# mulns/AccFlow

Hardware: AMD Instinct MI355X
Metric: frame-pairs/s (estimator pair-evals/s), AccFlow(RAFT) 7-frame 480x1024 backward accumulation (higher is better)
Workload: dtype f32 (direct-kernel operands split into 2 fp16 terms - activations kept pre-split in HBM as fp16 hi+lo, 4 B per element; other kernels 3 bf16 terms; f32 accumulate); 1 GPU; AccFlow(RAFT) 7-frame 480x1024, 12 GRU iters, 1 sequence(s)/GPU/step (BASELINE.json configs[2]; configs[3] when n_gpus=8); parallelism=1 rank, no process group: no collective runs, weights=deterministic random init (no checkpoints offline)

## Files before the change

accflow_amd/build.py:

```python
import os
import subprocess
import sys
from concurrent.futures import ThreadPoolExecutor

HERE = os.path.dirname(os.path.abspath(__file__))
ROOT = os.path.dirname(HERE)
CSRC = os.path.join(HERE, "csrc")
LIBDIR = os.path.join(HERE, "lib")
LIB = os.path.join(LIBDIR, "libaccflow_hip.so")
SOURCES = ["conv2d_f32.hip", "conv2d_f32_v1.hip", "conv2d_f32_v2.hip", "conv2d_f32_v3.hip", "conv2d_bf16s.hip", "conv2d_bf16s_v12.hip", "conv2d_bf16s_v11.hip", "conv2d_bf16s_v21.hip",
           "conv2d_direct_v_bf16x6.hip", "conv2d_direct_v_bf16n.hip", "conv2d_direct_v_f16.hip", "conv2d_direct_v_s16.hip", "conv2d_direct_v_s16tg.hip", "conv2d_direct_v_s16k.hip", "conv2d_direct_v_s16k9.hip",
           "conv2d_direct_v_f16n.hip", "conv2d_direct_v_bf16x3.hip", "conv_s16m_v0.hip", "conv_s16m_v1.hip", "conv_s16m_v2.hip",
           "conv_s16m_v3.hip", "conv2d_s16m.hip", "conv_stem.hip", "conv2d_direct.hip", "conv2d.hip", "corr_volume.hip",
           "corr_lookup.hip", "corr_disp.hip", "corr_alt.hip", "corr_lookup_conv.hip", "sampling.hip", "misc.hip", "gma.hip", "backward.hip"]
ARCH = "gfx950"


def _hipcc():
    for c in (os.environ.get("HIPCC"), "/opt/rocm/bin/hipcc", "hipcc"):
        if c and (os.path.isabs(c) and os.path.exists(c) or not os.path.isabs(c)):
            return c
    raise RuntimeError("hipcc not found")


def _newer(target, deps):
    if not os.path.exists(target):
        return False
    t = os.path.getmtime(target)
    return all(os.path.getmtime(d) <= t for d in deps)


def _deps(src, seen=None):
    import re
    seen = set() if seen is None else seen
    if src in seen:
        return seen
    seen.add(src)
    for name in re.findall(r'^\s*#\s*include\s+"([^"]+)"', open(src).read(), flags=re.M):
        for d in (os.path.dirname(src), CSRC, os.path.join(ROOT, "include")):
            cand = os.path.join(d, name)
            if os.path.exists(cand):
                _deps(cand, seen)
                break
    return seen


def build(force=False, verbose=False, libdir=None, defines=(), unit_defines=()):
    LIBDIR = libdir or globals()["LIBDIR"]
    LIB = os.path.join(LIBDIR, "libaccflow_hip.so")
    os.makedirs(LIBDIR, exist_ok=True)
    objdir = os.path.join(LIBDIR, "obj")
    os.makedirs(objdir, exist_ok=True)
    cc = _hipcc()
    flags = ["-O3", "--offload-arch=" + ARCH, "-fPIC", "-std=c++17", "-I" + os.path.join(ROOT, "include"),
             "-I" + CSRC, "-Wno-unused-result",
             "-mllvm", "-pragma-unroll-threshold=1000000"] + ["-D" + d for d in defines]
    jobs = []
    objs = []
    for s in SOURCES:
        src = os.path.join(CSRC, s)
        obj = os.path.join(objdir, s.replace(".hip", ".o"))
        objs.append(obj)
        extra = ["-D" + d for pre, d in unit_defines if s.startswith(pre)]
        if force or extra or not _newer(obj, sorted(_deps(src))):
            jobs.append([cc] + flags + extra + ["-c", src, "-o", obj])

    def run(cmd):
        import time
        if verbose:
            print(" ".join(cmd), flush=True)
        t0 = time.time()
        r = subprocess.run(cmd, capture_output=True, text=True)
        if r.returncode != 0:
            raise RuntimeError("hipcc failed: %s\n%s\n%s" % (" ".join(cmd), r.stdout, r.stderr))
        if verbose:
            print("  [%.0f s] %s" % (time.time() - t0, os.path.basename(cmd[-1])), flush=True)

    if jobs:
        with ThreadPoolExecutor(max_workers=min(8, len(jobs))) as ex:
            list(ex.map(run, jobs))
    if jobs or force or not os.path.exists(LIB):
        run([cc, "--offload-arch=" + ARCH, "-shared", "-fPIC", "-no-hip-rt", "-o", LIB] + objs)
    return LIB


if __name__ == "__main__":
    defs = [a[2:] for a in sys.argv[1:] if a.startswith("-D")]
    ld = [a.split("=", 1)[1] for a in sys.argv[1:] if a.startswith("--libdir=")]
    ud = [tuple(a.split("=", 1)[1].split(":", 1)) for a in sys.argv[1:] if a.startswith("--unit-define=")]
    print(build(force="--force" in sys.argv, verbose=True, libdir=ld[0] if ld else None, defines=defs, unit_defines=ud))
```

accflow_amd/csrc/conv2d.hip:

```cpp
#include "conv_common.h"

namespace {

__global__ void conv_pack_patch_kernel(const float* __restrict__ w, const float* __restrict__ scale, int Cout, int Cin,
                                       int T, int CoutPad, unsigned short* __restrict__ wp, int f16,
                                       const float* __restrict__ wscale16, int octs = 2,
                                       const float* __restrict__ gptr = nullptr) {
  const int nstep = (Cin + 8 * octs - 1) / (8 * octs) * T;
  const long long per_term = (long long)nstep * octs * CoutPad * 8;
  const long long idx = (long long)blockIdx.x * blockDim.x + threadIdx.x;
  if (idx >= per_term) return;
  const int q = (int)(idx & 7);
  long long r = idx >> 3;
  const int ch = (int)(r % CoutPad); r /= CoutPad;
  const int o = (int)(r % octs); r /= octs;
  const int step = (int)r, cc = step / T, tap = step % T;
  const int c = cc * 8 * octs + o * 8 + q;
  float val = 0.0f;
  if (c < Cin && ch < Cout) {
    val = w[((long long)ch * Cin + c) * T + tap];
    if (scale) val *= scale[ch];
    if (gptr) val *= gptr[0];
  }
  float rr = val;
  if (f16) {
    rr = val * (ldexpf(1.0f, -ACCFLOW_F16_ASHIFT) / wscale16[ch]);
#pragma unroll
    for (int t = 0; t < 3; ++t) {
      const _Float16 hq = t < 2 ? (_Float16)rr : (_Float16)0.0f;
      wp[t * per_term + idx] = __builtin_bit_cast(unsigned short, hq);
      rr -= (float)hq;
    }
    return;
  }
#pragma unroll
  for (int t = 0; t < 3; ++t) {
    const __bf16 bq = (__bf16)rr;
    wp[t * per_term + idx] = __builtin_bit_cast(unsigned short, bq);
    rr -= (float)bq;
  }
}

__global__ void conv_pack_bf16s_kernel(const float* __restrict__ w, const float* __restrict__ scale, int Cout, int Cin,
                                       int KH, int KW, int Kpad, int CoutPad, unsigned short* __restrict__ ws,
                                       int kmajor, float cscale, const float* __restrict__ gptr,
                                       const float* __restrict__ wscale16 = nullptr) {
  const long long idx = (long long)blockIdx.x * blockDim.x + threadIdx.x;
  if (idx >= (long long)Kpad * CoutPad) return;
  w += (long long)blockIdx.y * Cout * Cin * KH * KW;
  ws += (long long)blockIdx.y * 3 * Kpad * CoutPad;
  if (wscale16) wscale16 += (long long)blockIdx.y * CoutPad;
  const int k = (int)(idx / CoutPad), o = (int)(idx % CoutPad);
  const int T = KH * KW, K = Cin * T;
  float val = 0.0f;
  if (k < K && o < Cout) {
    const int c = k / T, t = k % T;
    val = kmajor ? w[(long long)k * Cout + o] : w[((long long)o * Cin + c) * T + t];
    if (scale) val *= scale[o];
    val *= cscale;
    if (gptr) val *= gptr[0];
  }
  const long long per_term = (long long)Kpad * CoutPad;
  const long long dst = ((long long)(k / 8) * CoutPad + o) * 8 + (k % 8);
  float r = val;
  if (wscale16) {
    r = val * (ldexpf(1.0f, -ACCFLOW_F16_ASHIFT) / wscale16[o]);
#pragma unroll
    for (int t = 0; t < 3; ++t) {
      const _Float16 hq = t < 2 ? (_Float16)r : (_Float16)0.0f;
      ws[t * per_term + dst] = __builtin_bit_cast(unsigned short, hq);
      r -= (float)hq;
    }
    return;
  }
#pragma unroll
  for (int t = 0; t < 3; ++t) {
    const __bf16 b = (__bf16)r;
    ws[t * per_term + dst] = __builtin_bit_cast(unsigned short, b);
    r -= (float)b;
  }
}

__global__ __launch_bounds__(256) void conv_pack_kmajor_kernel(const float* __restrict__ w, int Cout, int K, int Kpad,
// ... 771 lines not shown
}

extern "C" long long accflow_s16_item_words(int C, int H, int W) {
  return (long long)((C + 7) / 8) * 2 * H * W * 4;
}

extern "C" int accflow_conv_kpad(int Cin, int KH, int KW) {
  const int K = Cin * KH * KW;
  return (K + 31) / 32 * 32;
}

extern "C" int accflow_conv_coutpad(int Cout) { return (Cout + 127) / 128 * 128; }

extern "C" int accflow_conv_pack_f32(const float* w, const float* scale, int Cout, int Cin, int KH, int KW,
                                     int C0, int tap_major, float* wpack, int* ktab, void* stream) {
  if (!w || !wpack || !ktab || Cout <= 0 || Cin <= 0 || KH <= 0 || KW <= 0) return 1;
  const int Kpad = accflow_conv_kpad(Cin, KH, KW), CoutPad = accflow_conv_coutpad(Cout);
  const long long n = (long long)Kpad * CoutPad;
  hipLaunchKernelGGL(conv_pack_kernel, dim3(cdiv(n, 256)), dim3(256), 0, as_stream(stream), w, scale, Cout,
                     Cin, KH, KW, C0, tap_major, Kpad, CoutPad, wpack, reinterpret_cast<int4*>(ktab));
  ACCFLOW_RETURN_LAUNCH_STATUS();
}

extern "C" int accflow_conv_pack_all_f32(const float* w, const float* scale, int Cout, int Cin, int KH, int KW, int C0, int tap_major,
                                         int transpose_flip, float* wpack, int* ktab, void* wsplit, void* wpatch, void* wpatch16,
                                         float* wscale16, void* wsplit16, void* stream) {
  if (!w || !wpack || !ktab || Cout <= 0 || Cin <= 0 || KH <= 0 || KW <= 0) return 1;
  if ((wpatch16 || wsplit16) && !wscale16) return 1;
  if (tap_major && (wsplit || wpatch || wpatch16 || wsplit16)) return 1;
  const int Kpad = accflow_conv_kpad(Cin, KH, KW), CoutPad = accflow_conv_coutpad(Cout);
  hipLaunchKernelGGL(conv_pack_all_kernel, dim3(CoutPad), dim3(256), 0, as_stream(stream), w, scale, Cout, Cin, KH, KW, C0, tap_major,
                     transpose_flip, Kpad, CoutPad, wpack, reinterpret_cast<int4*>(ktab), reinterpret_cast<unsigned short*>(wsplit),
                     reinterpret_cast<unsigned short*>(wpatch), reinterpret_cast<unsigned short*>(wpatch16), wscale16,
                     reinterpret_cast<unsigned short*>(wsplit16));
  ACCFLOW_RETURN_LAUNCH_STATUS();
}

thread_local int* accflow_tls_dry_slots = nullptr;
thread_local int* accflow_tls_dry_route = nullptr;

extern "C" int accflow_conv_in_norm_supported(const accflow_conv_desc* desc) {
  if (!desc) return 0;
  int slots = 0, route = 0;
  accflow_conv_desc probe = *desc;
  probe.in_norm = nullptr;
  probe.stats = nullptr;
  accflow_tls_dry_slots = &slots;
  accflow_tls_dry_route = &route;
  const int rc = accflow_conv2d_f32(&probe, nullptr);
  accflow_tls_dry_slots = nullptr;
  accflow_tls_dry_route = nullptr;
  return rc ? 0 : route;
}

extern "C" int accflow_conv_stat_slots(const accflow_conv_desc* desc) {
  if (!desc || desc->epi != ACCFLOW_EPI_STORE || desc->act != ACCFLOW_ACT_NONE) return 0;
  int slots = 0;
  accflow_tls_dry_slots = &slots;
  const int rc = accflow_conv2d_f32(desc, nullptr);
  accflow_tls_dry_slots = nullptr;
  return rc ? 0 : slots;
}

bool accflow_conv_stem_eligible(const accflow_conv_desc& d);
int accflow_launch_conv_stem(const accflow_conv_desc& d, hipStream_t st);

extern "C" int accflow_conv_gru16_supported(void) {
  static const bool ok = [] {
    const char* a = getenv("ACCFLOW_DIRECT_KT"); const char* b = getenv("ACCFLOW_DIRECT_W4"); const char* c = getenv("ACCFLOW_S16M");
    return !(a && atoi(a) == 0) && !(b && atoi(b) == 0) && !(c && atoi(c) != 0);
  }();
  return ok ? 1 : 0;
}

extern "C" int accflow_conv2d_f32(const accflow_conv_desc* desc, void* stream) {
  if (!desc) return 1;
  accflow_conv_desc dd = *desc;
  if (dd.mode == ACCFLOW_CONV_F16X3 && (dd.wpatch16 || dd.wsplit16) && !dd.wscale16) return 1;
  if (dd.mode != ACCFLOW_CONV_F16X3) { dd.wpatch16 = nullptr; dd.wsplit16 = nullptr; }
  if (!dd.wpatch16 && !dd.wsplit16) dd.wscale16 = nullptr;
  dd.acc_scale = 0.0f;
  if (dd.nsrc < 0 || dd.nsrc > ACCFLOW_CONV_MAX_SRC) return 1;
  const bool gru16 = !dd.nsrc && dd.e0_fmt;
  if (gru16 && !(dd.in_fmt == (dd.in1 ? 3 : 1) && dd.e0 && dd.pre && dd.out16 && dd.mode == ACCFLOW_CONV_F16X3 && !dd.cb && !dd.kws &&
                 dd.KH * dd.KW == 5 && dd.stride == 1 && accflow_conv_gru16_supported() && !dd.stats &&
                 ((dd.epi == ACCFLOW_EPI_GRU_ZR && dd.p32 == 3 && dd.out && dd.Cout == 256) ||
                  (dd.epi == ACCFLOW_EPI_GRU_Q && dd.p32 == 6 && dd.e1 && dd.Cout == 128))))
    return 1;
  if (!gru16 && dd.p32 && !(dd.p32 == 1 && !dd.nsrc && dd.in_fmt == (dd.in1 ? 3 : 1) && dd.mode == ACCFLOW_CONV_F16X3 && dd.out && !dd.out16 &&
                            dd.epi == ACCFLOW_EPI_STORE && (dd.act == ACCFLOW_ACT_NONE || dd.act == ACCFLOW_ACT_RELU) && !dd.cb &&
                            !dd.kws && !dd.stats && dd.stride == 1 && (dd.Cout % 128) == 0 && accflow_conv_gru16_supported()))
    return 1;
  const bool multi = dd.nsrc > 0;
  if (multi) {
    if (dd.mode != ACCFLOW_CONV_F16X3 || !dd.wpatch16 || dd.in_norm || dd.offset || dd.wsplit_bs) return 1;
    dd.in_fmt = 0; dd.in0 = nullptr; dd.in1 = nullptr; dd.H = dd.OH; dd.W = dd.OW;
    dd.CoutPad = accflow_conv_coutpad(dd.Cout);
  }
  const accflow_conv_desc& d = dd;
  if ((!multi && (!d.in0 || !d.wpack || !d.ktab)) || d.B <= 0 || d.Cout <= 0 || d.OH <= 0 || d.OW <= 0) return 1;
  if (d.epi == ACCFLOW_EPI_TAPGEMM) {
    if (multi || d.mode != ACCFLOW_CONV_F16X3 || !d.wpatch16 || !d.wscale16 || d.in_fmt != (d.in1 ? 3 : 1) || d.act != ACCFLOW_ACT_RELU ||
        (d.Cout & 127) || d.kws || d.stats || d.in_norm || d.cb || d.pre || d.offset || !d.tg_w16 || !d.tg_scale || !d.tg_out ||
        d.tg_rows < 1 || d.tg_rows > ACCFLOW_TAPGEMM_MAXROWS || d.tg_coutpad < 32 || (d.tg_coutpad & 31) ||
        d.tg_out_bs < (long long)d.tg_rows * d.OH * d.OW || (d.Cout > 128 && d.tg_out_ps <= 0) || !accflow_conv_direct_eligible(d) ||
        d.Kpad != accflow_conv_kpad(d.C0 + d.C1, d.KH, d.KW) || d.CoutPad != accflow_conv_coutpad(d.Cout))
      return 1;
    if ((((long long)(d.B - 1)) * d.in0_bs + accflow_s16_item_words(d.C0, d.H, d.W)) * 4 >= (1LL << 32)) return 1;
    if (d.in1 && (((long long)(d.B - 1)) * d.in1_bs + accflow_s16_item_words(d.C1, d.H, d.W)) * 4 >= (1LL << 32)) return 1;
    return accflow_launch_conv_direct(d, 2, as_stream(stream));
  }
  if (!d.out && (!d.out16 || d.epi == ACCFLOW_EPI_GRU_ZR)) return 1;
  if (d.epi == ACCFLOW_EPI_GRU_ZR && !d.out2 && !d.out16) return 1;
  if ((d.in_fmt || d.out16) && d.mode != ACCFLOW_CONV_F16X3) return 1;
  if (d.in_fmt & ~3) return 1;
  if (d.out16) {
    const int ea = d.epi * 8 + d.act;
    if (ea != ACCFLOW_EPI_STORE * 8 + ACCFLOW_ACT_NONE && ea != ACCFLOW_EPI_STORE * 8 + ACCFLOW_ACT_RELU &&
        ea != ACCFLOW_EPI_STORE * 8 + ACCFLOW_ACT_SIGMOID && ea != ACCFLOW_EPI_RES_RELU * 8 + ACCFLOW_ACT_RELU &&
        ea != ACCFLOW_EPI_RES_RELU * 8 + ACCFLOW_ACT_NONE &&
        ea != ACCFLOW_EPI_GRU_ZR * 8 + ACCFLOW_ACT_SIGMOID && ea != ACCFLOW_EPI_GRU_Q * 8 + ACCFLOW_ACT_TANH &&
        ea != ACCFLOW_EPI_ACCUM * 8 + ACCFLOW_ACT_NONE)
      return 1;
  }
  if (d.cb && ((d.cb & 31) || (d.epi != ACCFLOW_EPI_STORE && d.epi != ACCFLOW_EPI_ACCUM) || d.stats || d.Cout % d.cb)) return 1;
  if (!multi && (d.Kpad != accflow_conv_kpad(d.C0 + d.C1, d.KH, d.KW) || d.CoutPad != accflow_conv_coutpad(d.Cout))) return 1;
  if ((d.epi == ACCFLOW_EPI_RES_RELU || d.epi == ACCFLOW_EPI_ACCUM) && !d.e0) return 1;
  if (d.epi == ACCFLOW_EPI_GRU_ZR && (!d.e0 || (d.Cout & 1))) return 1;
  if (d.epi == ACCFLOW_EPI_GRU_ZR && d.out16 && ((d.Cout >> 1) & 7)) return 1;
  if (d.epi == ACCFLOW_EPI_GRU_Q && (!d.e0 || !d.e1)) return 1;
  if (d.pre && d.epi != ACCFLOW_EPI_GRU_ZR && d.epi != ACCFLOW_EPI_GRU_Q) return 1;
  if (d.offset && !d.dmask) return 1;
  if ((long long)d.B * d.OH * d.OW >= (1LL << 31)) return 1;
  if (!multi) {
    const long long w0 = (d.in_fmt & 1) ? accflow_s16_item_words(d.C0, d.H, d.W) : (long long)d.C0 * d.H * d.W;
    const long long w1 = (d.in_fmt & 2) ? accflow_s16_item_words(d.C1, d.H, d.W) : (long long)d.C1 * d.H * d.W;
    if ((((long long)(d.B - 1)) * d.in0_bs + w0) * 4 >= (1LL << 32)) return 1;
    if (d.in1 && (((long long)(d.B - 1)) * d.in1_bs + w1) * 4 >= (1LL << 32)) return 1;
  }
  if (d.out16 && (((long long)(d.B - 1)) * d.out16_bs + accflow_s16_item_words(d.Cout, d.OH, d.OW)) * 4 >= (1LL << 32)) return 1;
  if (d.stats && (d.epi != ACCFLOW_EPI_STORE || d.act != ACCFLOW_ACT_NONE || d.stat_slots <= 0)) return 1;
  hipStream_t st = as_stream(stream);
  const long long Ptot = (long long)d.B * d.OH * d.OW;
  if (d.in_norm && !accflow_tls_dry_slots && !accflow_conv_in_norm_supported(&d)) return 1;
  if (d.stats && !accflow_tls_dry_slots) {
    int want = 0;
    accflow_tls_dry_slots = &want;
    accflow_conv_desc probe = d;
    probe.stats = nullptr;
    const int prc = accflow_conv2d_f32(&probe, nullptr);
    accflow_tls_dry_slots = nullptr;
    if (prc || want != d.stat_slots) return 1;
  }
  if (multi) return accflow_launch_conv_s16m(d, -1, st);
  static const bool stem_on = [] { const char* e = getenv("ACCFLOW_CONV_STEM"); return !e || atoi(e) != 0; }();
  if (stem_on && accflow_conv_stem_eligible(d)) return accflow_launch_conv_stem(d, st);
  static const bool s16m_on = [] { const char* e = getenv("ACCFLOW_S16M"); return e && atoi(e) != 0; }();
  if (d.in_fmt && s16m_on) {
    if (!accflow_conv_direct_eligible(d) || !d.wpatch16 || d.in_norm) return 1;
    if (d.in_fmt != (d.in1 ? 3 : 1)) return 1;
    accflow_conv_desc e = d;
    accflow_s16m_from_legacy(e);
    return accflow_launch_conv_s16m(e, -1, st);
  }
  if (d.in_fmt || d.out16 || d.cb) {
    if (!accflow_conv_direct_eligible(d) || !d.wpatch16 || d.stats || d.in_norm) return 1;
    if (d.in_fmt && d.in_fmt != (d.in1 ? 3 : 1)) return 1;
    return accflow_launch_conv_direct(d, d.Cout > 64 ? 2 : 1, st);
  }
  if (d.Cout <= 4 && !d.offset && (d.epi == ACCFLOW_EPI_STORE || d.epi == ACCFLOW_EPI_ACCUM || d.epi == ACCFLOW_EPI_RES_RELU)) {
    const bool same = d.stride == 1 && d.OH == d.H && d.OW == d.W && d.KH * d.KW >= 2 && d.C0 + d.C1 >= 16 &&
                      (8 + d.KH - 1) * (16 + d.KW - 1) <= 192 && d.KH * d.KW <= 25 && (!d.in1 || d.C0 % 16 == 0);
    ACCFLOW_DRY_RUN(0);
    if (same) {
      dim3 pgrid((unsigned)((long long)d.B * cdiv(d.OW, 16) * cdiv(d.OH, 8)));
      if (d.Cout <= 2) hipLaunchKernelGGL((conv2d_small_cout_patch_kernel<2>), pgrid, dim3(256), 0, st, d);
      else hipLaunchKernelGGL((conv2d_small_cout_patch_kernel<4>), pgrid, dim3(256), 0, st, d);
      ACCFLOW_RETURN_LAUNCH_STATUS();
    }
    dim3 grid(cdiv(Ptot, 64));
    if (d.Cout <= 2) hipLaunchKernelGGL((conv2d_small_cout_kernel<2>), grid, dim3(256), 0, st, d);
    else hipLaunchKernelGGL((conv2d_small_cout_kernel<4>), grid, dim3(256), 0, st, d);
    ACCFLOW_RETURN_LAUNCH_STATUS();
  }
  if (accflow_conv_direct_eligible(d)) {
    const long long nb = (long long)d.B * cdiv(d.OW, DIR_TW) * cdiv(d.OH, DIR_TH);
    const long long minb = (d.kws && (d.KH * d.KW >= 2 || d.C0 + d.C1 >= 512)) ? 0 : patch_min_blocks();
    if (d.Cout > 64 && nb * cdiv(d.Cout, 128) >= minb) return accflow_launch_conv_direct(d, 2, st);
    if (nb * cdiv(d.Cout, 64) >= minb) return accflow_launch_conv_direct(d, 1, st);
  }
  if (d.mode == ACCFLOW_CONV_F16X3 && !(d.wsplit16 && !d.offset && d.Cout > 32)) {
    accflow_conv_desc e = d;
    e.mode = ACCFLOW_CONV_BF16X6;
    e.wpatch = nullptr;
    e.wpatch16 = nullptr; e.wsplit16 = nullptr; e.wscale16 = nullptr;
    return accflow_conv2d_f32(&e, stream);
  }
  if (d.mode == ACCFLOW_CONV_F16X3 && d.wsplit_bs) {
    ACCFLOW_DRY_RUN(0);
    if ((d.OH * d.OW) % 64) return 1;
    return d.Cout > 64 ? accflow_launch_conv_bf16s(d, 2, 1, st) : accflow_launch_conv_bf16s(d, 1, 1, st);
  }
  if (d.mode == ACCFLOW_CONV_F16X3) {
    accflow_conv_desc e = d;
    e.wpatch16 = nullptr;
    auto nb = [&](int bc, int bp) { return (long long)cdiv(Ptot, bp) * cdiv(e.Cout, bc); };
    if (e.Cout <= 64) return nb(64, 128) >= 384 ? accflow_launch_conv_bf16s(e, 1, 2, st) : accflow_launch_conv_bf16s(e, 1, 1, st);
    if (nb(128, 128) >= 384) return accflow_launch_conv_bf16s(e, 2, 2, st);
    if (nb(128, 64) >= 384) return accflow_launch_conv_bf16s(e, 2, 1, st);
    return accflow_launch_conv_bf16s(e, 1, 1, st);
  }
  if (d.wsplit_bs) {
    ACCFLOW_DRY_RUN(0);
    if (d.mode == ACCFLOW_CONV_F32 || !d.wsplit || d.offset || ((d.OH * d.OW) % 64) || d.Cout <= 32) return 1;
// ... 27 lines not shown
```

accflow_amd/csrc/conv2d_direct.hip:

```cpp
#include "conv2d_direct_kernel.h"

namespace {

__global__ __launch_bounds__(256) void conv_ksplit_reduce_kernel(const accflow_conv_desc d, int Z) {
  const int OHW = d.OH * d.OW;
  const long long n = (long long)d.B * d.Cout * OHW;
  const long long i = (long long)blockIdx.x * 256 + threadIdx.x;
  if (i >= n) return;
  const int px = (int)(i % OHW);
  const int ch = (int)((i / OHW) % d.Cout);
  const int b = (int)(i / ((long long)OHW * d.Cout));
  float v = d.kws[i];
  for (int z = 1; z < Z; ++z) v += d.kws[(long long)z * n + i];
  v = fmaf(v, d.wscale16 ? d.wscale16[(d.wsplit_bs ? (long long)b * d.CoutPad : 0) + ch] : 1.0f, d.bias ? d.bias[ch] : 0.0f);
  if (d.pre && (d.epi == ACCFLOW_EPI_GRU_ZR || d.epi == ACCFLOW_EPI_GRU_Q)) v += d.pre[b * d.pre_bs + (long long)ch * OHW + px];
  v = apply_act(v, d.act);
  const long long o = (long long)ch * OHW + px;
  const int half = d.Cout >> 1;
  if (d.cb) {
    const int blk = ch / d.cb;
    const long long oc = (long long)(ch - blk * d.cb) * OHW + px;
    const float r = d.epi == ACCFLOW_EPI_ACCUM ? d.e0[b * d.e0_bs + blk * d.e0_cbs + oc] + v : v;
    d.out[b * d.out_bs + blk * d.out_cbs + oc] = r;
    return;
// ... 143 lines not shown
      } break;
      case ACCFLOW_EPI_ACCUM: t = d.e0[b * d.e0_bs + o] + t; break;
      default: break;
    }
    if (d.out) d.out[b * d.out_bs + o] = t;
    res[j] = t;
  }
  constexpr float ASC = (float)(1 << ACCFLOW_F16_ASHIFT);
  unsigned hi[2], lo[2];
  bool bad = false;
#pragma unroll
  for (int k = 0; k < 2; ++k) {
    const float a = res[2 * k] * ASC, c = res[2 * k + 1] * ASC;
    bad |= !(fabsf(a) < 65520.0f) | !(fabsf(c) < 65520.0f);
    const f32x2 v2 = {a, c};
    const f16x2 hq = __builtin_convertvector(v2, f16x2);
    const f32x2 back = __builtin_convertvector(hq, f32x2);
    const f32x2 rest = {a - back[0], c - back[1]};
    const f16x2 lq = __builtin_convertvector(rest, f16x2);
    hi[k] = __builtin_bit_cast(unsigned, hq);
    lo[k] = __builtin_bit_cast(unsigned, lq);
  }
  unsigned* base = reinterpret_cast<unsigned*>(d.out16) + b * d.out16_bs;
  int oct = q >> 1;
  const int w0 = (q & 1) * 2;
  if (d.cb) {
    base += (long long)((q * 4) / d.cb) * d.out16_cbs;
    oct = ((q * 4) % d.cb) >> 3;
  }
  unsigned* ph = base + (((long long)(oct * 2 + 0)) * OHW + px) * 4 + w0;
  unsigned* pl = base + (((long long)(oct * 2 + 1)) * OHW + px) * 4 + w0;
  typedef unsigned u2_ __attribute__((ext_vector_type(2)));
  *reinterpret_cast<u2_*>(ph) = u2_{hi[0], hi[1]};
  *reinterpret_cast<u2_*>(pl) = u2_{lo[0], lo[1]};
  if (bad && d.guard) atomicOr(d.guard, 1);
}

}

int conv_ksplit_reduce_launch(const accflow_conv_desc& d, int Z, hipStream_t st) {
  if (d.out16 && !(d.Cout & 7) && !(d.cb & 7) && d.epi != ACCFLOW_EPI_GRU_ZR) {
    const long long nthr = (long long)d.B * (d.Cout / 4) * d.OH * d.OW;
    hipLaunchKernelGGL(conv_ksplit_reduce_s16q_kernel, dim3(cdiv(nthr, 256)), dim3(256), 0, st, d, Z);
  } else if (d.out16) {
    const long long nthr = (long long)d.B * ((d.Cout + 7) / 8) * d.OH * d.OW;
    hipLaunchKernelGGL(conv_ksplit_reduce_s16_kernel, dim3(cdiv(nthr, 256)), dim3(256), 0, st, d, Z);
  } else {
    const long long nout = (long long)d.B * d.Cout * d.OH * d.OW;
    hipLaunchKernelGGL(conv_ksplit_reduce_kernel, dim3(cdiv(nout, 256)), dim3(256), 0, st, d, Z);
  }
  ACCFLOW_RETURN_LAUNCH_STATUS();
}

namespace {

template <int TC>
int launch_conv_direct(const accflow_conv_desc& d, hipStream_t st) {
  const int tiles = cdiv(d.OW, DIR_TW) * cdiv(d.OH, DIR_TH);
  const long long nb = (long long)d.B * tiles * cdiv(d.Cout, 2 * TC * 32);
  static const bool w4 = [] { const char* e = getenv("ACCFLOW_DIRECT_W4"); return !e || atoi(e) != 0; }();
  const bool norm_ok = !d.in1 && d.C0 <= DIR_NORM_MAXC && (TC == 1 || w4);
  if (accflow_tls_dry_route) *accflow_tls_dry_route = norm_ok ? 1 : 0;
  ACCFLOW_DRY_RUN(tiles * ((TC == 2 && w4) ? 1 : 2));
  if (d.in_norm && !norm_ok) return 1;
  int Z = 1;
  const long long nout = (long long)d.B * d.Cout * d.OH * d.OW;
  const int nchunk = (d.C0 + d.C1 + 15) / 16;
  if (d.kws && nchunk >= 256 && nb < 700 && !d.stats) {
    static const int zenv = [] { const char* e = getenv("ACCFLOW_DIRECT_KSPLIT"); return e ? atoi(e) : 0; }();
    double best = 0.0;
    for (int z = 1; z <= 8; ++z) {
      const double fill = (double)(nb * z) / (double)(cdiv(nb * z, 768) * 768);
      if (fill > best + 0.03) { best = fill; Z = z; }
    }
    if (zenv > 0) Z = zenv;
  } else if (d.kws && nb < 320 && !d.stats) {
    Z = (int)((512 + nb - 1) / nb);
    if (Z > 4) Z = 4;
    if (Z > nchunk / 2) Z = nchunk / 2;
  }
  if (Z > 1 && (long long)Z * nout > d.kws_elems) Z = (int)(d.kws_elems / nout);
  if (Z < 1) Z = 1;
  if (d.out16 && d.epi == ACCFLOW_EPI_GRU_ZR && ((d.Cout >> 1) & 7)) Z = 1;
  dim3 grid((unsigned)((long long)d.B * tiles), cdiv(d.Cout, 2 * TC * 32), Z);
  constexpr bool CAN_W4 = TC == 2;
  const bool f16 = d.mode == ACCFLOW_CONV_F16X3 && d.wpatch16;
  int rc;
  if (d.epi == ACCFLOW_EPI_TAPGEMM) {
    if (TC != 2 || !f16 || !d.in_fmt || Z != 1 || !(CAN_W4 && w4)) return 1;
    static const bool kt9_tg = [] { const char* e = getenv("ACCFLOW_DIRECT_KT9"); return !e || atoi(e) != 0; }();
    rc = (kt9_tg && d.KH == 3 && d.KW == 3 && (d.C0 + d.C1) % 16 == 0) ? accflow_direct_launch_s16k9(d, 2, true, grid, st)
                                                                        : accflow_direct_launch_s16tg(d, grid, st);
  } else if (d.in_fmt) {
    if (!f16 || d.in_norm || d.in_fmt != (d.in1 ? 3 : 1)) return 1;
    static const bool kt_on = [] { const char* e = getenv("ACCFLOW_DIRECT_KT"); return !e || atoi(e) != 0; }();
    static const bool kt9_on = [] { const char* e = getenv("ACCFLOW_DIRECT_KT9"); return !e || atoi(e) != 0; }();
    if (kt_on && TC == 2 && CAN_W4 && w4 && d.KH * d.KW == 5) rc = accflow_direct_launch_s16k(d, 5, grid, st);
    else if (kt9_on && (TC == 1 || (CAN_W4 && w4)) && d.KH == 3 && d.KW == 3) rc = accflow_direct_launch_s16k9(d, TC, false, grid, st);
    else rc = accflow_direct_launch_s16(d, TC, grid, st);
  } else if (d.in_norm) {
    rc = f16 ? accflow_direct_launch_f16_norm(d, TC, grid, st)
             : accflow_direct_launch_bf16_norm(d, TC, d.mode == ACCFLOW_CONV_BF16X3 ? 2 : 3, grid, st);
  } else {
    rc = f16 ? accflow_direct_launch_f16(d, TC, CAN_W4 && w4, grid, st)
             : accflow_direct_launch_bf16(d, TC, d.mode == ACCFLOW_CONV_BF16X3 ? 2 : 3, CAN_W4 && w4, grid, st);
  }
  if (rc) return rc;
  if (Z > 1) return conv_ksplit_reduce_launch(d, Z, st);
  ACCFLOW_RETURN_LAUNCH_STATUS();
}

}

template <int NT, bool F16>
__global__ __launch_bounds__(256, 2) void corr_disp_gemm_kernel(const accflow_conv_desc d) {
  constexpr int TC = 2, TP = 2;
  __shared__ __attribute__((aligned(16))) unsigned char smem[DISP2_LDS_BYTES];
#ifdef ACCFLOW_KPROF
  const unsigned long long tL0 = __builtin_amdgcn_s_memrealtime();
#endif
  const int tid = threadIdx.x, lane = tid & 63;
  const int wave = __builtin_amdgcn_readfirstlane(tid >> 6);
  const int wc = wave >> 1, wp = wave & 1;
  const int l31 = lane & 31, kh = lane >> 5;
  const int P = d.OH * d.OW;
  const int npb = (P + 127) >> 7, percol = (npb + 7) >> 3;
  const int xcd = blockIdx.x & 7, seq = blockIdx.x >> 3;
  const int pb = xcd + 8 * (seq % percol), qt = seq / percol;
  if (pb >= npb) return;
  const int ncx = (d.OW + 63) >> 6;
  const int yo = qt / ncx, xc = qt - yo * ncx;
  const int cblk0 = pb * 128;
  const int nstep = d.Kpad / 16;
  const long long step_bytes = 2LL * d.CoutPad * 16, term_bytes = (long long)(d.Kpad / 8) * d.CoutPad * 16;
  const __amdgpu_buffer_rsrc_t ra = __builtin_amdgcn_make_buffer_rsrc(
      const_cast<void*>(F16 ? d.wpatch16 : d.wpatch), 0, (int)(unsigned)(3 * term_bytes), 0x00020000);
  const __amdgpu_buffer_rsrc_t rb = __builtin_amdgcn_make_buffer_rsrc(
      const_cast<float*>(d.in0), 0, (int)(unsigned)(3 * term_bytes), 0x00020000);
  const unsigned avoff = (unsigned)((kh * d.CoutPad + cblk0 + wc * 64 + l31) * 16);
  unsigned bvoff[2];
#pragma unroll
  for (int i = 0; i < 2; ++i) {
    const int y2 = 2 * yo + wp, x2 = xc * 64 + i * 32 + l31;
    bvoff[i] = (y2 < d.OH && x2 < d.OW) ? (unsigned)((kh * d.CoutPad + y2 * d.OW + x2) * 16) : 0xFFFFFFFFu;
  }
#define CG_LOAD(STEP, A, Bf)                                                                                     \
  _Pragma("unroll") for (int t = 0; t < NT; ++t) _Pragma("unroll") for (int i = 0; i < 2; ++i) {                 \
    const int so = (int)(unsigned)(t * term_bytes + (STEP) * step_bytes);                                        \
    A[t][i] = __builtin_bit_cast(bf16x8, __builtin_amdgcn_raw_buffer_load_b128(ra, (int)(avoff + i * 512), so, 0)); \
    Bf[t][i] = __builtin_bit_cast(bf16x8, __builtin_amdgcn_raw_buffer_load_b128(rb, (int)bvoff[i], so, 0));      \
  }
  f32x16 acc[TC][TP];
#pragma unroll
  for (int tc = 0; tc < TC; ++tc)
#pragma unroll
    for (int tp = 0; tp < TP; ++tp)
#pragma unroll
      for (int r = 0; r < 16; ++r) acc[tc][tp][r] = 0.0f;
  constexpr int PD = NT == 2 ? 2 : 1;
  bf16x8 aA[NT][TC], bA[NT][TP], aB[NT][TC], bB[NT][TP], aC[NT][TC], bC[NT][TP];
  CG_LOAD(0, aA, bA);
  if (PD == 2 && nstep > 1) { CG_LOAD(1, aB, bB); }
#define CG_STEP(STEP, AC, BC, AN, BN)                                                                            \
  do {                                                                                                           \
    if ((STEP) + PD < nstep) { CG_LOAD((STEP) + PD, AN, BN); }                                                   \
    constexpr int NPAIR = NT == 3 ? 6 : 3;                                                                       \
// ... 282 lines not shown
    constexpr int PA[3] = {1, 0, 0}, PB[3] = {0, 1, 0};
#pragma unroll
    for (int pr = 0; pr < 3; ++pr)
#pragma unroll
      for (int tc = 0; tc < TC; ++tc)
#pragma unroll
        for (int tp = 0; tp < TP; ++tp) {
          if (ACCFLOW_CORR_ABL & 2) acc[tc][tp][pr] += __builtin_bit_cast(float, __builtin_bit_cast(u32x4, A[PA[pr]][tc])[0] ^ __builtin_bit_cast(u32x4, Bf[PB[pr]][tp])[1]);
          else acc[tc][tp] = dir_mfma<true>(A[PA[pr]][tc], Bf[PB[pr]][tp], acc[tc][tp]);
        }
  }
  __syncthreads();
  if ((ACCFLOW_CORR_ABL & 8) && acc[0][0][0] != 12345.678f) return;
#ifdef ACCFLOW_KPROF
  __builtin_amdgcn_sched_barrier(0);
  const unsigned long long tL1 = __builtin_amdgcn_s_memrealtime();
#endif
  corr_disp_store2(d, acc, reinterpret_cast<float*>(smem), reinterpret_cast<int*>(smem) + 64 * DISP_PITCH,
                   reinterpret_cast<float*>(smem + DISP_LDS_BYTES), d.out2, cblk0, yo, xc, wc, wp, lane, wave, tid);
#ifdef ACCFLOW_KPROF
  __builtin_amdgcn_sched_barrier(0);
  const unsigned long long tL2 = __builtin_amdgcn_s_memrealtime();
  asm volatile("s_waitcnt vmcnt(0)" ::: "memory");
  if (tid == 0) {
    const int slot = (blockIdx.x & 4095) * 16;
    g_kprof[slot + 8] = tL1 - tL0;
    g_kprof[slot + 9] = tL2 - tL1;
    g_kprof[slot + 11] = __builtin_amdgcn_s_memrealtime() - tL0;
    g_kprof[slot + 10] = 1;
  }
#endif
}

int accflow_launch_corr_disp_direct(const accflow_conv_desc& d, hipStream_t st) {
  const int P = d.OH * d.OW, npb = cdiv(P, 128);
  if (!d.out2) return 1;
  const int nqt = cdiv(d.OH, 2) * cdiv(d.OW, 64);
  dim3 grid(8 * ((npb + 7) / 8) * nqt);
  static const bool ringk = [] { const char* e = getenv("ACCFLOW_CORR_GEMM"); return !(e && e[0] == 'r'); }();
  if (d.mode == ACCFLOW_CONV_F16X3 && d.wpatch16 && ringk) {
    hipLaunchKernelGGL(corr_disp_ring_kernel, grid, dim3(256), 0, st, d);
  } else if (d.mode == ACCFLOW_CONV_F16X3 && d.wpatch16) hipLaunchKernelGGL((corr_disp_gemm_kernel<2, true>), grid, dim3(256), 0, st, d);
  else if (d.mode == ACCFLOW_CONV_BF16X3) hipLaunchKernelGGL((corr_disp_gemm_kernel<2, false>), grid, dim3(256), 0, st, d);
  else hipLaunchKernelGGL((corr_disp_gemm_kernel<3, false>), grid, dim3(256), 0, st, d);
  ACCFLOW_RETURN_LAUNCH_STATUS();
}

int accflow_launch_conv_direct(const accflow_conv_desc& d, int tc, hipStream_t st) {
  const bool pointwise = d.epi == ACCFLOW_EPI_STORE || d.epi == ACCFLOW_EPI_RES_RELU || d.epi == ACCFLOW_EPI_ACCUM;
  if (tc == 2 && d.Cout > 128 && d.Cout % 128 > 0 && d.Cout % 128 <= 64 && pointwise && !d.stats && !accflow_tls_dry_slots && !(d.kws && (long long)d.B * cdiv(d.OW, DIR_TW) * cdiv(d.OH, DIR_TH) * cdiv(d.Cout, 128) < 320)) {
    const int ch0 = d.Cout / 128 * 128;
    const long long OHW = (long long)d.OH * d.OW;
    accflow_conv_desc a = d, b = d;
    a.Cout = ch0;
    b.Cout = d.Cout - ch0;
    b.out = d.out ? d.out + ch0 * OHW : nullptr;
    if (d.bias) b.bias = d.bias + ch0;
    if (d.wscale16) b.wscale16 = d.wscale16 + ch0;
    if (d.e0) b.e0 = d.e0 + ch0 * OHW;
    if (d.out16) b.out16 = reinterpret_cast<char*>(d.out16) + (long long)(ch0 / 8) * 2 * OHW * 16;
    if (d.wpatch) b.wpatch = reinterpret_cast<const char*>(d.wpatch) + (long long)ch0 * 16;
    if (d.wpatch16) b.wpatch16 = reinterpret_cast<const char*>(d.wpatch16) + (long long)ch0 * 16;
    const int rc = launch_conv_direct<2>(a, st);
    if (rc) return rc;
    return launch_conv_direct<1>(b, st);
  }
  return tc == 2 ? launch_conv_direct<2>(d, st) : launch_conv_direct<1>(d, st);
}

bool accflow_conv_direct_eligible(const accflow_conv_desc& d) {
  if (!d.wpatch || d.wsplit_bs || d.mode == ACCFLOW_CONV_F32 || d.offset || d.stride != 1 || d.Cout <= 4) return false;
  if (d.OH != d.H || d.OW != d.W) return false;
  if ((DIR_TH + d.KH - 1) * (DIR_TW + d.KW - 1) > DIR_NPMAX) return false;
  if (d.C0 + d.C1 < 16) return false;
  if (d.in1 && (d.C0 % (d.KH * d.KW == 1 ? 32 : 16))) return false;
  return true;
}

#ifdef ACCFLOW_KPROF
#define ACCFLOW_DIRECT_UNITY
#include "conv2d_direct_v_s16.hip"
#include "conv2d_direct_v_s16tg.hip"
#include "conv2d_direct_v_s16k.hip"
#include "conv2d_direct_v_s16k9.hip"
#include "conv2d_direct_v_f16.hip"
#include "conv2d_direct_v_f16n.hip"
#include "conv2d_direct_v_bf16x6.hip"
#include "conv2d_direct_v_bf16x3.hip"
#include "conv2d_direct_v_bf16n.hip"
extern "C" int accflow_debug_occupancy(int* out) {
  int n = 0;
  hipOccupancyMaxActiveBlocksPerMultiprocessor(&out[n++], conv2d_direct_bf16s_kernel<2, 3>, 256, 0);
  hipOccupancyMaxActiveBlocksPerMultiprocessor(&out[n++], conv2d_direct_bf16s_kernel<2, 2, true>, 256, 0);
  hipOccupancyMaxActiveBlocksPerMultiprocessor(&out[n++], conv2d_direct_bf16s_kernel<1, 3>, 256, 0);
  hipDeviceProp_t pr; hipGetDeviceProperties(&pr, 0);
  out[n++] = (int)(pr.maxSharedMemoryPerMultiProcessor / 1024); out[n++] = (int)(pr.sharedMemPerBlock / 1024);
  out[n++] = pr.regsPerMultiprocessor; out[n++] = pr.regsPerBlock;
  return n;
}
extern "C" int accflow_debug_kprof(unsigned long long* out, int reset) {
  hipDeviceSynchronize();
  hipMemcpyFromSymbol(out, HIP_SYMBOL(g_kprof), 4096 * 16 * 8);
  if (reset) { void* p; hipGetSymbolAddress(&p, HIP_SYMBOL(g_kprof)); hipMemset(p, 0, 4096 * 16 * 8); }
  return (int)hipGetLastError();
}
#endif
```

accflow_amd/csrc/conv2d_direct_kernel.h:

```cpp
#pragma once
#include "conv_common.h"
#include <utility>

namespace {


#ifndef ACCFLOW_DIRECT_LEAN
#define ACCFLOW_DIRECT_LEAN 1
#endif
#ifndef ACCFLOW_DIRECT_LEAN_MAXSTEPS
#define ACCFLOW_DIRECT_LEAN_MAXSTEPS 0
#endif
#ifndef ACCFLOW_F16_PAIRMASK
#define ACCFLOW_F16_PAIRMASK 7
#endif
#ifndef ACCFLOW_DIRECT_KT_BUPFRONT
#define ACCFLOW_DIRECT_KT_BUPFRONT 0
#endif
#ifndef ACCFLOW_DIRECT_KT_WAVES
#define ACCFLOW_DIRECT_KT_WAVES 3
#endif
#ifndef ACCFLOW_DIRECT_SETPRIO
#define ACCFLOW_DIRECT_SETPRIO 0
#endif
// ... 33 lines not shown
template <bool F16, class PixMap>
__device__ __forceinline__ void conv_epilogue_tapgemm(const accflow_conv_desc& d, f32x16 (&acc)[1][4], int cblk0, int wave,
                                                      int lane, int tid, int OHW, PixMap pixmap, float* red) {
  typedef float f32x4_ __attribute__((ext_vector_type(4)));
  typedef float f32x2_ __attribute__((ext_vector_type(2)));
  typedef _Float16 f16x2_ __attribute__((ext_vector_type(2)));
  const int l31 = lane & 31, kh = lane >> 5, lh4 = kh * 4;
  const int rowbase = cblk0 + wave * 32;
  const int R = d.tg_rows;
  const __amdgpu_buffer_rsrc_t r_b = __builtin_amdgcn_make_buffer_rsrc(const_cast<float*>(d.bias ? d.bias : d.wscale16), 0,
                                                                      d.bias ? d.Cout * 4 : 0, 0x00020000);
  const __amdgpu_buffer_rsrc_t r_s = __builtin_amdgcn_make_buffer_rsrc(const_cast<float*>(d.wscale16), 0, d.CoutPad * 4, 0x00020000);
  f32x4_ bv[4], sv[4];
#pragma unroll
  for (int m = 0; m < 4; ++m) {
    const int off = (rowbase + 8 * m + lh4) * 4;
    bv[m] = __builtin_bit_cast(f32x4_, __builtin_amdgcn_raw_buffer_load_b128(r_b, off, 0, 0));
    sv[m] = __builtin_bit_cast(f32x4_, __builtin_amdgcn_raw_buffer_load_b128(r_s, off, 0, 0));
  }
  const long long step_bytes2 = 2LL * d.tg_coutpad * 16, term_bytes2 = (long long)(d.Cout >> 4) * step_bytes2;
  const __amdgpu_buffer_rsrc_t r_w2 = __builtin_amdgcn_make_buffer_rsrc(const_cast<void*>(d.tg_w16), 0,
                                                                       (int)(unsigned)(2 * term_bytes2), 0x00020000);
  const unsigned av2 = (unsigned)((kh * d.tg_coutpad + l31) * 16);
  bf16x8 a2[2][2];
#pragma unroll
  for (int s = 0; s < 2; ++s)
#pragma unroll
    for (int t = 0; t < 2; ++t)
      a2[s][t] = __builtin_bit_cast(bf16x8, __builtin_amdgcn_raw_buffer_load_b128(
                                               r_w2, (int)av2, (int)(unsigned)(t * term_bytes2 + ((rowbase >> 4) + s) * step_bytes2), 0));
  constexpr float ASC16 = (float)(1 << ACCFLOW_F16_ASHIFT);
  bool bad16 = false;
#pragma unroll
  for (int tp = 0; tp < 4; ++tp) {
    f32x16 z2;
#pragma unroll
    for (int r = 0; r < 16; ++r) z2[r] = 0.0f;
#pragma unroll
    for (int s = 0; s < 2; ++s) {
      unsigned hi[4], lo[4];
#pragma unroll
      for (int e2 = 0; e2 < 4; ++e2) {
        const int m = 2 * s + (e2 >> 1), q = (2 * e2) & 3;
        float va = fmaf(acc[0][tp][4 * m + q], sv[m][q], bv[m][q]) + 0.0f;
        float vb = fmaf(acc[0][tp][4 * m + q + 1], sv[m][q + 1], bv[m][q + 1]) + 0.0f;
        va = fmaxf(va, 0.0f) * ASC16;
        vb = fmaxf(vb, 0.0f) * ASC16;
        bad16 |= !(va < 65520.0f) | !(vb < 65520.0f);
        const f32x2_ v2 = {va, vb};
        const f16x2_ hq = __builtin_convertvector(v2, f16x2_);
        const f32x2_ back = __builtin_convertvector(hq, f32x2_);
        const f32x2_ rest = {va - back[0], vb - back[1]};
        const f16x2_ lq = __builtin_convertvector(rest, f16x2_);
        hi[e2] = __builtin_bit_cast(unsigned, hq);
        lo[e2] = __builtin_bit_cast(unsigned, lq);
      }
      const u32x4 hv = {hi[0], hi[1], hi[2], hi[3]}, lv = {lo[0], lo[1], lo[2], lo[3]};
      const bf16x8 bh = __builtin_bit_cast(bf16x8, hv), bl = __builtin_bit_cast(bf16x8, lv);
      z2 = dir_mfma<F16>(a2[s][1], bh, z2);
      z2 = dir_mfma<F16>(a2[s][0], bl, z2);
      z2 = dir_mfma<F16>(a2[s][0], bh, z2);
    }
#pragma unroll
    for (int r = 0; r < 16; ++r) {
      const int row = 8 * (r >> 2) + lh4 + (r & 3);
      if (row < R) red[(wave * R + row) * (DIR_TH * DIR_TW) + tp * 32 + l31] = z2[r];
    }
  }
  if (bad16 && d.guard) atomicOr(d.guard, 1);
  __syncthreads();
  const long long obase = (long long)(cblk0 >> 7) * d.tg_out_ps;
  constexpr int NPX = DIR_TH * DIR_TW;
  for (int o = tid; o < R * NPX; o += 256) {
    const int row = o / NPX, px = o - row * NPX;
    const float v = ((red[o] + red[R * NPX + o]) + red[2 * R * NPX + o]) + red[3 * R * NPX + o];
    int b;
    const int rem = pixmap(px, b);
    if (rem >= 0) d.tg_out[obase + (long long)b * d.tg_out_bs + (long long)row * OHW + rem] = v * d.tg_scale[row];
  }
}

constexpr int DIR_NORM_MAXC = 256;
template <int TC, int NT, bool F16 = false, bool W4 = false, bool NORM = false, bool S16 = false, int PM = 7, bool TG = false, int KT = 0,
          int KWC = 0>
__global__ __launch_bounds__(256, (KT == 5 ? ACCFLOW_DIRECT_KT_WAVES : 2)) void conv2d_direct_bf16s_kernel(const accflow_conv_desc d) {
  static_assert(!F16 || NT == 2, "the fp16 split has two terms");
  static_assert(KT == 0 || ((S16 || (F16 && NORM)) && (KT & 1)), "the tap-specialised loop: S16 sources or the fp16 normalise-on-load gather, an odd tap count");
  static_assert(!TG || (W4 && S16 && PM == 7), "ACCFLOW_EPI_TAPGEMM: the 4 x 1 wave layout over S16 sources");
  static_assert(!W4 || TC == 2, "the 4 x 1 wave layout is the 128-channel kernel's");
  static_assert(!S16 || (F16 && !NORM), "S16 sources hold the fp16 split");
#ifdef ACCFLOW_KPROF
  const unsigned long long tL0 = __builtin_amdgcn_s_memrealtime();
  unsigned long long kp[8] = {0, 0, 0, 0, 0, 0, 0, 0};
#endif
  constexpr int WC = W4 ? 4 : 2, WP = W4 ? 1 : 2, TP = W4 ? 4 : 2, OCT = 2;
  constexpr int TCW = W4 ? 1 : TC;
  constexpr int BC = WC * TCW * 32;
  static_assert(BC == 2 * TC * 32 && DIR_TH * DIR_TW == WP * TP * 32, "4 x 32 pixel tile = 128 accumulator columns");
  constexpr int PSTAGE = NT * OCT * DIR_NPMAX;
  constexpr int TGWORDS = TG ? 4 * ACCFLOW_TAPGEMM_MAXROWS * DIR_TH * DIR_TW / 4 : 0;
  __shared__ u32x4 Pst[2 * PSTAGE > TGWORDS ? 2 * PSTAGE : TGWORDS];
  __shared__ float Nrm[NORM ? 2 * DIR_NORM_MAXC : 2];

  const int tid = threadIdx.x, lane = tid & 63;
  const int wave = __builtin_amdgcn_readfirstlane(tid >> 6);
  const int wc = wave / WP, wp = wave % WP;
  const int l31 = lane & 31, kh = lane >> 5;
  int bx = blockIdx.x, by = blockIdx.y;
#if ACCFLOW_CONV_XCD_ORDER
  if (gridDim.y > 1 && (d.C0 + d.C1) * d.KH * d.KW >= ACCFLOW_CONV_XCD_MIN_K) {
    const int X = gridDim.x, Y = gridDim.y, L = bx + X * by, full = X & ~7;
    if (L < full * Y) {
      const int G = L / (8 * Y), r = L - G * 8 * Y;
      by = r >> 3;
      bx = G * 8 + (r & 7);
    } else {
      const int r = L - full * Y, rem = X - full;
      by = r / rem;
      bx = full + r - by * rem;
    }
  }
#endif
  const int cblk0 = by * BC;
  const int OHW = d.OH * d.OW;
  const int tilesX = (d.OW + DIR_TW - 1) / DIR_TW, tilesY = (d.OH + DIR_TH - 1) / DIR_TH;
  const int tb = bx / (tilesX * tilesY), trem = bx - tb * tilesX * tilesY;
  const int oy0 = (trem / tilesX) * DIR_TH, ox0 = (trem % tilesX) * DIR_TW;
#ifdef ACCFLOW_DIRECT_STAGGER
  if (KT == 5 && (blockIdx.x & 1)) {
    for (int i = 0; i < ACCFLOW_DIRECT_STAGGER; ++i) __builtin_amdgcn_s_sleep(127);
  }
#endif
  const int T = d.KH * d.KW;
  const int PW = DIR_TW + d.KW - 1, NP = (DIR_TH + d.KH - 1) * PW;
  const int Cin = d.C0 + d.C1;
  const bool wide = T == 1;
  const int CCH = wide ? 32 : 16;
  const int NOCT = wide ? 4 : 2;
  const int NPS = wide ? DIR_NPMAX / 2 : DIR_NPMAX;
  const int TPC = wide ? 2 : T;
  const int nstep = (Cin + 15) / 16 * T, nchunk = (Cin + CCH - 1) / CCH;
  const int HW = d.H * d.W;
  const int c_begin = (int)((long long)nchunk * blockIdx.z / gridDim.z);
  const int c_end = (int)((long long)nchunk * (blockIdx.z + 1) / gridDim.z);
  const int step_end = min(c_end * TPC, nstep);

  unsigned voff0[2], voff1[2];
  int p_oct[2], p_pix[2];
#pragma unroll
  for (int i = 0; i < 2; ++i) {
    const int it = tid + 256 * i;
    const bool live = it < NOCT * NP;
    p_oct[i] = live ? it / NP : 0;
    p_pix[i] = live ? it - p_oct[i] * NP : 0;
    const int py = p_pix[i] / PW, px = p_pix[i] - py * PW;
    const int iy = oy0 - d.padH + py, ix = ox0 - d.padW + px;
    const bool ok = live && (unsigned)iy < (unsigned)d.H && (unsigned)ix < (unsigned)d.W;
    voff0[i] = ok ? (unsigned)(((long long)tb * d.in0_bs + iy * d.W + ix) * 4) : 0xFFFFFFFFu;
    voff1[i] = ok ? (unsigned)(((long long)tb * d.in1_bs + iy * d.W + ix) * 4) : 0xFFFFFFFFu;
    if (!live) p_pix[i] = -1;
  }
  const __amdgpu_buffer_rsrc_t rsrc0 = __builtin_amdgcn_make_buffer_rsrc(
      const_cast<float*>(d.in0), 0, (int)(unsigned)((((long long)(d.B - 1)) * d.in0_bs + (long long)d.C0 * HW) * 4),
      0x00020000);
  const __amdgpu_buffer_rsrc_t rsrc1 = __builtin_amdgcn_make_buffer_rsrc(
      const_cast<float*>(d.in1 ? d.in1 : d.in0), 0,
      (int)(unsigned)(d.in1 ? (((long long)(d.B - 1)) * d.in1_bs + (long long)d.C1 * HW) * 4 : 0), 0x00020000);
  unsigned pixo[4] = {0xFFFFFFFFu, 0xFFFFFFFFu, 0xFFFFFFFFu, 0xFFFFFFFFu};
  const int O0 = (d.C0 + 7) >> 3, O1 = (d.C1 + 7) >> 3;
  const __amdgpu_buffer_rsrc_t rs16_0 = __builtin_amdgcn_make_buffer_rsrc(
      const_cast<float*>(d.in0), 0, (int)(unsigned)((((long long)(d.B - 1)) * d.in0_bs + (long long)O0 * 2 * HW * 4) * 4),
      0x00020000);
  const __amdgpu_buffer_rsrc_t rs16_1 = __builtin_amdgcn_make_buffer_rsrc(
      const_cast<float*>(d.in1 ? d.in1 : d.in0), 0,
      (int)(unsigned)(d.in1 ? (((long long)(d.B - 1)) * d.in1_bs + (long long)O1 * 2 * HW * 4) * 4 : 0), 0x00020000);
  if constexpr (S16) {
#pragma unroll
    for (int q = 0; q < 4; ++q) {
      const int pp = q * 64 + lane;
      const int py = pp / PW, px = pp - py * PW;
      const int iy = oy0 - d.padH + py, ix = ox0 - d.padW + px;
      const bool ok = pp < NP && (unsigned)iy < (unsigned)d.H && (unsigned)ix < (unsigned)d.W;
      pixo[q] = ok ? (unsigned)(iy * d.W + ix) * 16u : 0xFFFFFFFFu;
    }
  }
  auto issue_dma = [&](int stage, int cc) {
    const int c0 = cc * CCH;
    const bool second = c0 >= d.C0;
    const int cs = second ? c0 - d.C0 : c0, osrc = second ? O1 : O0;
    const long long bs = second ? d.in1_bs : d.in0_bs;
    const unsigned item = (unsigned)((long long)tb * bs * 4);
#pragma unroll
    for (int i = 0; i < 4; ++i) {
      const int row = wide ? 2 * wave + (i >> 1) : wave;
      const int q = wide ? (i & 1) : i;
      if (!wide && q * 64 >= NP) continue;
      const int t = wide ? row >> 2 : row >> 1, o = wide ? row & 3 : row & 1;
      const int oct = (cs >> 3) + o;
      const unsigned soff = (unsigned)__builtin_amdgcn_readfirstlane((int)(item + (unsigned)((oct * 2 + t) * HW) * 16u));
      const unsigned voff = oct < osrc ? (q == 0 ? pixo[0] : q == 1 ? pixo[1] : q == 2 ? pixo[2] : pixo[3]) : 0xFFFFFFFFu;
      const int slot = __builtin_amdgcn_readfirstlane(stage * PSTAGE + t * (OCT * DIR_NPMAX) + o * NPS + q * 64);
      if (second)
        __builtin_amdgcn_raw_ptr_buffer_load_lds(rs16_1, (__attribute__((address_space(3))) void*)&Pst[slot], 16, (int)voff,
                                                 (int)soff, 0, 0);
      else
        __builtin_amdgcn_raw_ptr_buffer_load_lds(rs16_0, (__attribute__((address_space(3))) void*)&Pst[slot], 16, (int)voff,
                                                 (int)soff, 0, 0);
    }
  };
  float xa[8], xb[8];
  unsigned vq0[2], vq1[2];
#pragma unroll
  for (int i = 0; i < 2; ++i) {
    const unsigned po = (unsigned)p_oct[i] * 8u * (unsigned)HW * 4u;
    vq0[i] = voff0[i] != 0xFFFFFFFFu ? voff0[i] + po : 0xFFFFFFFFu;
    vq1[i] = voff1[i] != 0xFFFFFFFFu ? voff1[i] + po : 0xFFFFFFFFu;
  }
  auto gather_patch = [&](int cc) {
    const int c0 = cc * CCH;
    const bool second = c0 >= d.C0;
    const __amdgpu_buffer_rsrc_t rs = second ? rsrc1 : rsrc0;
    const int cs = second ? c0 - d.C0 : c0, cmax = second ? d.C1 : d.C0;
    if (cs + CCH <= cmax) {
      const unsigned va = second ? vq1[0] : vq0[0], vb = second ? vq1[1] : vq0[1];
      const unsigned so = (unsigned)__builtin_amdgcn_readfirstlane(cs) * (unsigned)HW * 4u;
#pragma unroll
      for (int q = 0; q < 8; ++q) {
        const int sq = (int)(so + (unsigned)q * (unsigned)HW * 4u);
        xa[q] = __builtin_bit_cast(float, __builtin_amdgcn_raw_buffer_load_b32(rs, (int)va, sq, 0));
        xb[q] = __builtin_bit_cast(float, __builtin_amdgcn_raw_buffer_load_b32(rs, (int)vb, sq, 0));
      }
      return;
    }
#pragma unroll
    for (int q = 0; q < 8; ++q) {
      const int ca = cs + p_oct[0] * 8 + q, cb = cs + p_oct[1] * 8 + q;
      const unsigned va = second ? voff1[0] : voff0[0], vb = second ? voff1[1] : voff0[1];
      const unsigned oa = (ca < cmax && va != 0xFFFFFFFFu) ? va + (unsigned)ca * (unsigned)HW * 4u : 0xFFFFFFFFu;
      const unsigned ob = (cb < cmax && vb != 0xFFFFFFFFu) ? vb + (unsigned)cb * (unsigned)HW * 4u : 0xFFFFFFFFu;
      xa[q] = __builtin_bit_cast(float, __builtin_amdgcn_raw_buffer_load_b32(rs, (int)oa, 0, 0));
      xb[q] = __builtin_bit_cast(float, __builtin_amdgcn_raw_buffer_load_b32(rs, (int)ob, 0, 0));
    }
  };
  bool bad = false;
  constexpr float ASC = (float)(1 << ACCFLOW_F16_ASHIFT);
  if constexpr (NORM) {
    for (int i = tid; i < 2 * d.C0; i += 256) Nrm[i] = d.in_norm[(long long)tb * 2 * d.C0 + i];
    __syncthreads();
  }
  auto store_patch = [&](int stage, int cc) {
    if constexpr (NORM) {
      const int ca = cc * CCH + p_oct[0] * 8, cb = cc * CCH + p_oct[1] * 8;
      const bool ina = voff0[0] != 0xFFFFFFFFu, inb = voff0[1] != 0xFFFFFFFFu;
#pragma unroll
      for (int q = 0; q < 8; ++q) {
        const bool oka = ina && ca + q < d.C0, okb = inb && cb + q < d.C0;
        const float ma = Nrm[2 * min(ca + q, d.C0 - 1)], ra = Nrm[2 * min(ca + q, d.C0 - 1) + 1];
        const float mb = Nrm[2 * min(cb + q, d.C0 - 1)], rb = Nrm[2 * min(cb + q, d.C0 - 1) + 1];
        xa[q] = oka ? fmaxf((xa[q] - ma) * ra, 0.0f) : 0.0f;
        xb[q] = okb ? fmaxf((xb[q] - mb) * rb, 0.0f) : 0.0f;
      }
    }
    u32x4 terms[NT];
    if constexpr (F16) split8_f16<0>(xa, terms, bad, ASC);
    else split8_bf16<NT, 0>(xa, terms);
    if (p_pix[0] >= 0) {
#pragma unroll
      for (int t = 0; t < NT; ++t) Pst[stage * PSTAGE + t * (OCT * DIR_NPMAX) + p_oct[0] * NPS + p_pix[0]] = terms[t];
    }
    if constexpr (F16) split8_f16<0>(xb, terms, bad, ASC);
    else split8_bf16<NT, 0>(xb, terms);
    if (p_pix[1] >= 0) {
#pragma unroll
      for (int t = 0; t < NT; ++t) Pst[stage * PSTAGE + t * (OCT * DIR_NPMAX) + p_oct[1] * NPS + p_pix[1]] = terms[t];
    }
  };

  const long long step_bytes = 2LL * d.CoutPad * 16, term_bytes = (long long)nstep * step_bytes;
  const __amdgpu_buffer_rsrc_t rsrcw = __builtin_amdgcn_make_buffer_rsrc(const_cast<void*>(F16 ? d.wpatch16 : d.wpatch), 0,
                                                                        (int)(unsigned)(3 * term_bytes), 0x00020000);
  const unsigned avoff = (unsigned)((kh * d.CoutPad + cblk0 + wc * TCW * 32 + l31) * 16);
#define DIR_LOAD_A(STEP, A)                                                                                      \
  _Pragma("unroll") for (int t = 0; t < NT; ++t) _Pragma("unroll") for (int tc = 0; tc < TCW; ++tc)              \
      A[t][tc] = __builtin_bit_cast(bf16x8, __builtin_amdgcn_raw_buffer_load_b128(                              \
          rsrcw, (int)(avoff + tc * 512), (int)(unsigned)(t * term_bytes + (STEP) * step_bytes), 0))

  int pbase[TP];
#pragma unroll
  for (int tp = 0; tp < TP; ++tp) pbase[tp] = (wp * TP + tp) * PW + l31;

  f32x16 acc[TCW][TP];
#pragma unroll
  for (int tc = 0; tc < TCW; ++tc)
#pragma unroll
    for (int tp = 0; tp < TP; ++tp)
#pragma unroll
      for (int r = 0; r < 16; ++r) acc[tc][tp][r] = 0.0f;

  bf16x8 aA[NT][TCW], aB[NT][TCW];
  DIR_LOAD_A(c_begin * TPC, aA);
  if constexpr (S16) {
    issue_dma(c_begin & 1, c_begin);
    asm volatile("s_waitcnt vmcnt(0)" ::: "memory");
  } else {
    gather_patch(c_begin);
    store_patch(c_begin & 1, c_begin);
  }
  __syncthreads();

  int cc = c_begin, tap = 0, ty = 0, tx = 0;
#define DIR_STEP(STEP, ACUR, ANXT)                                                                               \
  do {                                                                                                           \
    KPROF_T(tA);                                                                                                 \
    const int pstage = cc & 1;                                                                                   \
    const bool next_chunk = cc + 1 < c_end;                                                                      \
    if ((STEP) + 1 < step_end) { DIR_LOAD_A((STEP) + 1, ANXT); }                                                 \
    if (tap == 0 && next_chunk) {                                                                                \
      if constexpr (S16) issue_dma(pstage ^ 1, cc + 1); else gather_patch(cc + 1);                               \
    }                                                                                                            \
    KPROF_T(tA1);                                                                                                \
    const int toff = wide ? tap * 2 * NPS : ty * PW + tx;                                                        \
    bf16x8 b[NT][TP];                                                                                            \
    _Pragma("unroll") for (int t = 0; t < NT; ++t) _Pragma("unroll") for (int tp = 0; tp < TP; ++tp)             \
        b[t][tp] = __builtin_bit_cast(bf16x8, Pst[pstage * PSTAGE + t * (OCT * DIR_NPMAX) + kh * NPS + pbase[tp] + toff]); \
    KPROF_T(tB);                                                                                                 \
    KPROF_WAIT();                                                                                                \
    KPROF_T(tB2);                                                                                                \
    {                                                                                                            \
      if (ACCFLOW_DIRECT_SETPRIO) __builtin_amdgcn_s_setprio(ACCFLOW_DIRECT_SETPRIO);                            \
      constexpr int NPAIR = NT == 3 ? 6 : 3;                                                                     \
      constexpr int PA[6] = {2, 0, 1, 1, 0, 0}, PB[6] = {0, 2, 1, 0, 1, 0};                                      \
      _Pragma("unroll") for (int pr = 6 - NPAIR; pr < 6; ++pr) _Pragma("unroll") for (int tc = 0; tc < TCW; ++tc) \
          _Pragma("unroll") for (int tp = 0; tp < TP; ++tp) if (!F16 || (((ACCFLOW_F16_PAIRMASK & PM) >> (pr - 3)) & 1))  \
              acc[tc][tp] = dir_mfma<F16>(ACUR[PA[pr]][tc], b[PB[pr]][tp], acc[tc][tp]);                         \
      if (ACCFLOW_DIRECT_SETPRIO) __builtin_amdgcn_s_setprio(0);                                                 \
    }                                                                                                            \
    KPROF_T(tC);                                                                                                 \
    if (++tx == d.KW) { tx = 0; ++ty; }                                                                          \
    if (++tap == TPC || (STEP) + 1 == step_end) {                                                                \
      if constexpr (S16) { asm volatile("s_waitcnt vmcnt(0)" ::: "memory"); }                                    \
      else { if (next_chunk) store_patch(pstage ^ 1, cc + 1); }                                                  \
      KPROF_T(tD);                                                                                               \
      __syncthreads();                                                                                           \
      KPROF_T(tE);                                                                                               \
      KPROF_ACC(3, tD - tC); KPROF_ACC(4, tE - tD);                                                              \
      tap = 0; ty = 0; tx = 0; ++cc;                                                                             \
    }                                                                                                            \
    KPROF_ACC(0, tA1 - tA); KPROF_ACC(7, tB - tA1); KPROF_ACC(1, tB2 - tB); KPROF_ACC(2, tC - tB2); KPROF_ACC(5, 1); \
  } while (0)

#ifdef ACCFLOW_KPROF
  const unsigned long long tK0 = __builtin_readcyclecounter();
  const unsigned long long tR0 = __builtin_amdgcn_s_memrealtime();
  if (tid == 0) KP_SLOT(14) = tR0 - tL0;
#endif
  if constexpr (KT > 0) {
    static_assert(KWC > 0 && KT % KWC == 0, "the tap-specialised loop knows the kernel's width");
    constexpr int PWC_ = DIR_TW + KWC - 1;
    s16m_i32x4 wdesc;
    {
      const unsigned long long wp_ = (unsigned long long)(F16 ? d.wpatch16 : d.wpatch);
      wdesc[0] = (int)(unsigned)wp_;
      wdesc[1] = (int)(unsigned)((wp_ >> 32) & 0xFFFFu);
      wdesc[2] = (int)(unsigned)(3 * term_bytes);
      wdesc[3] = 0x00020000;
    }
    constexpr int NPC = (DIR_TH + KT / KWC - 1) * PWC_;
    constexpr int NDMA = !S16 ? 16 : (NPC + 63) / 64 < 4 ? (NPC + 63) / 64 : 4;
    auto load_a_asm = [&](int step, bf16x8 (&A)[NT][TCW]) __attribute__((always_inline)) {
#pragma unroll
      for (int t = 0; t < NT; ++t)
#pragma unroll
        for (int tc = 0; tc < TCW; ++tc)
        {
          u32x4 frag;
          s16m_load_a(frag, avoff + tc * 512, wdesc,
                      __builtin_amdgcn_readfirstlane((int)(unsigned)(t * term_bytes + (long long)step * step_bytes)));
          A[t][tc] = __builtin_bit_cast(bf16x8, frag);
        }
    };
    constexpr int PWC = DIR_TW + KWC - 1;
    const u32x4* const pb0 = &Pst[kh * DIR_NPMAX + wp * TP * PWC + l31];
    auto chunk = [&](int cq, bf16x8 (&A0)[NT][TCW], bf16x8 (&A1)[NT][TCW]) __attribute__((always_inline)) {
      const int pstage = cq & 1;
      const bool next_chunk = cq + 1 < c_end;
      const int sbase = cq * KT;
      const u32x4* const pb = pb0 + pstage * PSTAGE;
      dir_static_for<KT>([&](auto tap_) {
        constexpr int TAP = decltype(tap_)::value;
        bf16x8 (&ACUR)[NT][TCW] = (TAP & 1) ? A1 : A0;
        bf16x8 (&ANXT)[NT][TCW] = (TAP & 1) ? A0 : A1;
        const int snext = sbase + TAP + 1;
        if constexpr (TAP + 1 < KT) { load_a_asm(snext, ANXT); }
        else { if (next_chunk) { load_a_asm(snext, ANXT); } }
        if constexpr (TAP == 0) {
          if (next_chunk) {
            if constexpr (S16) issue_dma(pstage ^ 1, cq + 1);
            else gather_patch(cq + 1);
          }
        }
        bf16x8 b[NT][TP];
#pragma unroll
        for (int tt = 0; tt < NT; ++tt)
#pragma unroll
          for (int tp = 0; tp < TP; ++tp)
            b[tt][tp] = __builtin_bit_cast(bf16x8, pb[tt * (OCT * DIR_NPMAX) + tp * PWC + (TAP / KWC) * PWC + TAP % KWC]);
        constexpr int PA[3] = {1, 0, 0}, PB[3] = {0, 1, 0};
#pragma unroll
        for (int pr = 0; pr < 3; ++pr)
#pragma unroll
          for (int tc = 0; tc < TCW; ++tc)
#pragma unroll
            for (int tp = 0; tp < TP; ++tp) acc[tc][tp] = dir_mfma<F16>(ACUR[PA[pr]][tc], b[PB[pr]][tp], acc[tc][tp]);
#if ACCFLOW_DIRECT_KT_BUPFRONT
        __builtin_amdgcn_sched_group_barrier(0x100, NT * TP, 0);
        __builtin_amdgcn_sched_group_barrier(0x008, 3 * TCW * TP, 0);
#endif
        __builtin_amdgcn_sched_barrier(0);
        if constexpr (TAP == 0 && KT > 1) { if (next_chunk) s16m_wait_vm<NDMA>(); else s16m_wait_vm<0>(); }
        else if constexpr (TAP + 1 < KT) { s16m_wait_vm<0>(); }
      });
      s16m_wait_vm<0>();
      if constexpr (!S16) { if (next_chunk) store_patch(pstage ^ 1, cq + 1); }
      __syncthreads();
    };
    for (int cq = c_begin; cq < c_end; cq += 2) {
      chunk(cq, aA, aB);
      if (cq + 1 < c_end) chunk(cq + 1, aB, aA);
    }
  } else {
  for (int step = c_begin * TPC; step < step_end; step += 2) {
    DIR_STEP(step, aA, aB);
    if (step + 1 < step_end) DIR_STEP(step + 1, aB, aA);
  }
  }
#undef DIR_STEP
#undef DIR_LOAD_A
#ifdef ACCFLOW_KPROF
  {
    const unsigned long long tK1 = __builtin_readcyclecounter();
    if (tid == 0) {
      for (int i = 0; i < 6; ++i) KP_SLOT(i) = kp[i];
      KP_SLOT(6) = tK1 - tK0;
      KP_SLOT(7) = kp[7];
      KP_SLOT(8) = __builtin_amdgcn_s_memrealtime() - tR0;
      KP_SLOT(10) = 1;
    }
  }
#endif
  if constexpr (F16) {
    if (bad && d.guard) atomicOr(d.guard, 1);
  }
  auto pixmap = [&](int j, int& b) {
    const int oy = oy0 + j / DIR_TW, ox = ox0 + j % DIR_TW;
    b = tb;
    return (oy < d.OH && ox < d.OW) ? oy * d.OW + ox : -1;
  };
  if constexpr (TG) {
    conv_epilogue_tapgemm<F16>(d, acc, cblk0, wave, lane, tid, OHW, pixmap, reinterpret_cast<float*>(Pst));
    return;
  }
  if (gridDim.z > 1) {
    accflow_conv_desc e = d;
    e.out = d.kws + (long long)blockIdx.z * d.B * d.Cout * OHW;
    e.out_bs = (long long)d.Cout * OHW;
    e.bias = nullptr;
    e.wscale16 = nullptr;
    e.out16 = nullptr;
    e.cb = 0;
    conv_epilogue_impl<ACCFLOW_EPI_STORE, ACCFLOW_ACT_NONE, WC, WP, TCW, TP>(e, acc, cblk0, wc, wp, lane, OHW, pixmap);
    return;
  }
  if constexpr (S16) {
    if ((ACCFLOW_DIRECT_LEAN || d.p32 || nstep <= ACCFLOW_DIRECT_LEAN_MAXSTEPS) && d.epi == ACCFLOW_EPI_STORE && !d.cb && !d.stats && cblk0 + (wc + 1) * TCW * 32 <= d.Cout &&
        (d.act == ACCFLOW_ACT_NONE || d.act == ACCFLOW_ACT_RELU)) {
      if (d.act == ACCFLOW_ACT_RELU) conv_epilogue_lean<ACCFLOW_ACT_RELU, WC, WP, TCW, TP>(d, acc, cblk0, wc, wp, lane, OHW, pixmap);
      else conv_epilogue_lean<ACCFLOW_ACT_NONE, WC, WP, TCW, TP>(d, acc, cblk0, wc, wp, lane, OHW, pixmap);
      return;
    }
  }
#ifdef ACCFLOW_DIRECT_ABL_NOEPI
  if ((d.epi == ACCFLOW_EPI_GRU_ZR || d.epi == ACCFLOW_EPI_GRU_Q) && acc[0][0][0] != 12345.678f) return;
#endif
  if constexpr (S16 && W4 && KT == 5) {
    if (d.e0_fmt) {
      if (d.epi == ACCFLOW_EPI_GRU_ZR) conv_epilogue_gru16<true, TP>(d, acc, cblk0, wc, lane, OHW, pixmap);
      else conv_epilogue_gru16<false, TP>(d, acc, cblk0, wc, lane, OHW, pixmap);
      return;
    }
  }
  conv_epilogue_px<WC, WP, TCW, TP, decltype(pixmap), F16>(d, acc, cblk0, wc, wp, lane, OHW, pixmap, tb, trem * WP + wp);
#ifdef ACCFLOW_KPROF
  __builtin_amdgcn_sched_barrier(0);
  const unsigned long long tS = __builtin_amdgcn_s_memrealtime();
  asm volatile("s_waitcnt vmcnt(0)" ::: "memory");
  if (tid == 0) {
    KP_SLOT(15) = tS - tL0;
    KP_SLOT(11) = __builtin_amdgcn_s_memrealtime() - tL0;
  }
#endif
}


}

int accflow_direct_launch_s16(const accflow_conv_desc& d, int tc, dim3 grid, hipStream_t st);
int accflow_direct_launch_s16tg(const accflow_conv_desc& d, dim3 grid, hipStream_t st);
int accflow_direct_launch_s16k9(const accflow_conv_desc& d, int tc, bool tapgemm, dim3 grid, hipStream_t st);
int accflow_direct_launch_s16k(const accflow_conv_desc& d, int kt, dim3 grid, hipStream_t st);
int accflow_direct_launch_f16(const accflow_conv_desc& d, int tc, bool w4, dim3 grid, hipStream_t st);
int accflow_direct_launch_f16_norm(const accflow_conv_desc& d, int tc, dim3 grid, hipStream_t st);
int accflow_direct_launch_bf16(const accflow_conv_desc& d, int tc, int nt, bool w4, dim3 grid, hipStream_t st);
int accflow_direct_launch_bf16_norm(const accflow_conv_desc& d, int tc, int nt, dim3 grid, hipStream_t st);
```

accflow_amd/csrc/conv_common.h:

```cpp
#pragma once
#include "common.h"
#include <stdlib.h>

int accflow_launch_conv_f32(const accflow_conv_desc& d, int wc, int wp, int tc, int tp, hipStream_t st);
int accflow_launch_conv_bf16s(const accflow_conv_desc& d, int tc, int tp, hipStream_t st);
int conv_ksplit_reduce_launch(const accflow_conv_desc& d, int Z, hipStream_t st);
int accflow_launch_corr_disp_bf16s(const accflow_conv_desc& d, hipStream_t st);
int accflow_launch_corr_disp_direct(const accflow_conv_desc& d, hipStream_t st);
int accflow_launch_conv_direct(const accflow_conv_desc& d, int tc, hipStream_t st);
bool accflow_conv_direct_eligible(const accflow_conv_desc& d);
int accflow_launch_conv_s16m(const accflow_conv_desc& d, int lay, hipStream_t st);
void accflow_s16m_from_legacy(accflow_conv_desc& e);
extern thread_local int* accflow_tls_dry_slots;
extern thread_local int* accflow_tls_dry_route;
#define ACCFLOW_DRY_RUN(SLOTS)                                 \
  do {                                                         \
    if (accflow_tls_dry_slots) {                               \
      *accflow_tls_dry_slots = (SLOTS);                        \
      return 0;                                                \
    }                                                          \
  } while (0)
#ifndef ACCFLOW_EPI_GRU_AHEAD
#define ACCFLOW_EPI_GRU_AHEAD 3
#endif
// ... 295 lines not shown
    const int rem = pixmap(wp * TP * 32 + tp * 32 + l31, b);
    const bool ok = rem >= 0;
    vo_16[tp] = ok && has16 ? (unsigned)((b * d.out16_bs + (long long)rem * 4) * 4 + lh4 * 2) : MASKED;
    vo_out[tp] = !(ok && has32) ? MASKED
                 : (d.p32 & 1) ? (unsigned)((b * d.out_bs + (long long)rem * 8 + lh4) * 4)
                               : (unsigned)((b * d.out_bs + (long long)rem + (long long)lh4 * OHW) * 4);
  }
  const bool p32o = (d.p32 & 1) != 0;
  typedef float f32x4_ __attribute__((ext_vector_type(4)));
  typedef unsigned u32x4_ __attribute__((ext_vector_type(4)));
  f32x4_ bv[TC][4], sv[TC][4];
#pragma unroll
  for (int tc = 0; tc < TC; ++tc)
#pragma unroll
    for (int m = 0; m < 4; ++m) {
      const int off = (rowbase + tc * 32 + 8 * m + lh4) * 4;
      bv[tc][m] = __builtin_bit_cast(f32x4_, __builtin_amdgcn_raw_buffer_load_b128(r_b, off, 0, 0));
      sv[tc][m] = __builtin_bit_cast(f32x4_, __builtin_amdgcn_raw_buffer_load_b128(r_s, off, 0, 0));
    }
  const bool no_scale = d.wscale16 == nullptr;
  bool bad16 = false;
  typedef float f32x2_ __attribute__((ext_vector_type(2)));
  typedef _Float16 f16x2_ __attribute__((ext_vector_type(2)));
  typedef unsigned u32x2_ __attribute__((ext_vector_type(2)));
  constexpr float ASC16 = (float)(1 << ACCFLOW_F16_ASHIFT);
#pragma unroll
  for (int tc = 0; tc < TC; ++tc)
#pragma unroll
    for (int m = 0; m < 4; ++m) {
      float o[TP][4];
#pragma unroll
      for (int q = 0; q < 4; ++q) {
        const int r = 4 * m + q;
        const float s = no_scale ? 1.0f : sv[tc][m][q];
        const int so = (rowbase + tc * 32 + 8 * m + q) * OHW4;
#pragma unroll
        for (int tp = 0; tp < TP; ++tp) {
          float v = fmaf(acc[tc][tp][r], s, bv[tc][m][q]) + 0.0f;
          if (ACT == ACCFLOW_ACT_RELU) v = fmaxf(v, 0.0f);
          o[tp][q] = v;
#ifndef ACCFLOW_KPROF_NOSTORE
          if (!p32o) __builtin_amdgcn_raw_buffer_store_b32(__builtin_bit_cast(unsigned, v), r_out, (int)vo_out[tp], so, 0);
#endif
        }
      }
      if (p32o) {
        const int so32 = ((rowbase + tc * 32 + 8 * m) >> 3) * OHW * 32;
#pragma unroll
        for (int tp = 0; tp < TP; ++tp) {
          const u32x4_ pv = {__builtin_bit_cast(unsigned, o[tp][0]), __builtin_bit_cast(unsigned, o[tp][1]),
                             __builtin_bit_cast(unsigned, o[tp][2]), __builtin_bit_cast(unsigned, o[tp][3])};
          __builtin_amdgcn_raw_buffer_store_b128(pv, r_out, (int)vo_out[tp], so32, 0);
        }
      }
      if (has16) {
        const int so16 = ((rowbase + tc * 32 + 8 * m) >> 3) * 2 * OHW * 16;
#pragma unroll
        for (int tp = 0; tp < TP; ++tp) {
          unsigned hi2[2], lo2[2];
#pragma unroll
          for (int k = 0; k < 2; ++k) {
            const float a = o[tp][2 * k] * ASC16, b = o[tp][2 * k + 1] * ASC16;
            bad16 |= !(fabsf(a) < 65520.0f) | !(fabsf(b) < 65520.0f);
            const f32x2_ v2 = {a, b};
            const f16x2_ hq = __builtin_convertvector(v2, f16x2_);
            const f32x2_ back = __builtin_convertvector(hq, f32x2_);
            const f32x2_ rest = {a - back[0], b - back[1]};
            const f16x2_ lq = __builtin_convertvector(rest, f16x2_);
            hi2[k] = __builtin_bit_cast(unsigned, hq);
            lo2[k] = __builtin_bit_cast(unsigned, lq);
          }
          const u32x2_ hv = {hi2[0], hi2[1]}, lv = {lo2[0], lo2[1]};
#ifndef ACCFLOW_KPROF_NOSTORE
          __builtin_amdgcn_raw_buffer_store_b64(hv, r_o16, (int)vo_16[tp], so16, 0);
          __builtin_amdgcn_raw_buffer_store_b64(lv, r_o16, (int)vo_16[tp], so16 + OHW * 16, 0);
#endif
        }
      }
    }
  if (has16 && bad16 && d.guard) atomicOr(d.guard, 1);
}


template <bool ZR, int TP, class PixMap>
__device__ __forceinline__ void conv_epilogue_gru16(const accflow_conv_desc& d, f32x16 (&acc)[1][TP], int cblk0, int wc, int lane,
                                                    int OHW, PixMap pixmap) {
  static_assert(TP == 4, "the 4 x 1 wave layout: 32 channels x 128 pixels per wave");
  constexpr unsigned MASKED = 0xFFFFFFFFu;
  constexpr int TPH = 2;
  typedef float f32x4_ __attribute__((ext_vector_type(4)));
  typedef float f32x2_ __attribute__((ext_vector_type(2)));
  typedef _Float16 f16x2_ __attribute__((ext_vector_type(2)));
  typedef unsigned u32x2_ __attribute__((ext_vector_type(2)));
  typedef unsigned u32x4_ __attribute__((ext_vector_type(4)));
  const int l31 = lane & 31, lh4 = (lane >> 5) * 4;
  const int rowbase = cblk0 + wc * 32;
  const int half = d.Cout >> 1;
  const bool zrow = ZR && rowbase < half;
  const bool need_h = !zrow;
  const int nst = ZR ? half : d.Cout;
  const int cst = ZR ? rowbase - half : rowbase;
  auto rng = [&](long long bs, int nch) { return (int)(unsigned)((((long long)(d.B - 1)) * bs + (long long)nch * OHW) * 4); };
  const __amdgpu_buffer_rsrc_t r_pre = __builtin_amdgcn_make_buffer_rsrc(const_cast<float*>(d.pre), 0, rng(d.pre_bs, d.Cout), 0x00020000);
  const __amdgpu_buffer_rsrc_t r_z = __builtin_amdgcn_make_buffer_rsrc(ZR ? (float*)d.out : const_cast<float*>(d.e1), 0,
                                                                      ZR ? rng(d.out_bs, half) : rng(d.e1_bs, d.Cout), 0x00020000);
  const int s16rng = (int)(unsigned)((((long long)(d.B - 1)) * d.e0_bs + (long long)((nst + 7) >> 3) * 2 * OHW * 4) * 4);
  const __amdgpu_buffer_rsrc_t r_h = __builtin_amdgcn_make_buffer_rsrc(const_cast<float*>(d.e0), 0, s16rng, 0x00020000);
  const __amdgpu_buffer_rsrc_t r_o16 = __builtin_amdgcn_make_buffer_rsrc(
      d.out16, 0, (int)(unsigned)((((long long)(d.B - 1)) * d.out16_bs + (long long)((nst + 7) >> 3) * 2 * OHW * 4) * 4), 0x00020000);
  const __amdgpu_buffer_rsrc_t r_b = __builtin_amdgcn_make_buffer_rsrc(const_cast<float*>(d.bias ? d.bias : d.wscale16), 0,
                                                                      d.bias ? d.Cout * 4 : 0, 0x00020000);
  const __amdgpu_buffer_rsrc_t r_s = __builtin_amdgcn_make_buffer_rsrc(const_cast<float*>(d.wscale16), 0, d.CoutPad * 4, 0x00020000);
  constexpr float ASC16 = (float)(1 << ACCFLOW_F16_ASHIFT);
  bool bad16 = false;
#pragma unroll
  for (int hh = 0; hh < TP / TPH; ++hh) {
    unsigned vo_p[TPH], vo_z[TPH], vo_h[TPH], vo_o[TPH];
#pragma unroll
    for (int t = 0; t < TPH; ++t) {
      int b;
      const int rem = pixmap((hh * TPH + t) * 32 + l31, b);
      const bool ok = rem >= 0;
      vo_p[t] = ok ? (unsigned)((b * d.pre_bs + (long long)rem * 8 + lh4) * 4) : MASKED;
      vo_z[t] = ok ? (unsigned)((b * (ZR ? d.out_bs : d.e1_bs) + (long long)rem * 8 + lh4) * 4) : MASKED;
      vo_h[t] = ok ? (unsigned)((b * d.e0_bs + (long long)rem * 4) * 4 + lh4 * 2) : MASKED;
      vo_o[t] = ok ? (unsigned)((b * d.out16_bs + (long long)rem * 4) * 4 + lh4 * 2) : MASKED;
    }
    f32x4_ pre[2][TPH], zz[2][TPH], bv[2], sv[2];
    u32x2_ hhi[2][TPH], hlo[2][TPH];
#define GRU16_FETCH(M, S)                                                                                          \
    do {                                                                                                           \
      const int ch_ = rowbase + 8 * (M);                             \
      bv[S] = __builtin_bit_cast(f32x4_, __builtin_amdgcn_raw_buffer_load_b128(r_b, (ch_ + lh4) * 4, 0, 0));       \
      sv[S] = __builtin_bit_cast(f32x4_, __builtin_amdgcn_raw_buffer_load_b128(r_s, (ch_ + lh4) * 4, 0, 0));       \
      const int sop_ = (ch_ >> 3) * OHW * 32;                           \
      const int so16_ = ((cst + 8 * (M)) >> 3) * 2 * OHW * 16;                   \
      _Pragma("unroll") for (int t = 0; t < TPH; ++t) {                                                            \
        pre[S][t] = __builtin_bit_cast(f32x4_, __builtin_amdgcn_raw_buffer_load_b128(r_pre, (int)vo_p[t], sop_, 0)); \
        if (!ZR) zz[S][t] = __builtin_bit_cast(f32x4_, __builtin_amdgcn_raw_buffer_load_b128(r_z, (int)vo_z[t], sop_, 0)); \
        if (need_h) {                                                                                              \
          hhi[S][t] = __builtin_bit_cast(u32x2_, __builtin_amdgcn_raw_buffer_load_b64(r_h, (int)vo_h[t], so16_, 0)); \
          hlo[S][t] = __builtin_bit_cast(u32x2_, __builtin_amdgcn_raw_buffer_load_b64(r_h, (int)vo_h[t], so16_ + OHW * 16, 0)); \
        }                                                                                                          \
      }                                                                                                            \
    } while (0)
    GRU16_FETCH(0, 0);
#pragma unroll
    for (int m = 0; m < 4; ++m) {
      const int S = m & 1;
      if (m + 1 < 4) GRU16_FETCH(m + 1, S ^ 1);
#pragma unroll
      for (int t = 0; t < TPH; ++t) {
        const int tp = hh * TPH + t;
        float o[4];
#pragma unroll
        for (int q = 0; q < 4; ++q) {
          const float v = apply_act(fmaf(acc[0][tp][4 * m + q], sv[S][q], bv[S][q]) + pre[S][t][q],
                                    ZR ? ACCFLOW_ACT_SIGMOID : ACCFLOW_ACT_TANH);
          if (need_h) {
            const unsigned wh = hhi[S][t][q >> 1], wl = hlo[S][t][q >> 1];
            const unsigned short hq = (unsigned short)((q & 1) ? wh >> 16 : wh & 0xFFFFu), lq = (unsigned short)((q & 1) ? wl >> 16 : wl & 0xFFFFu);
            const float hv = ((float)__builtin_bit_cast(_Float16, hq) + (float)__builtin_bit_cast(_Float16, lq)) * (1.0f / ASC16);
            o[q] = ZR ? v * hv : gru_blend(zz[S][t][q], hv, v);
          } else {
            o[q] = v;
          }
        }
        if (zrow) {
          const u32x4_ pv = {__builtin_bit_cast(unsigned, o[0]), __builtin_bit_cast(unsigned, o[1]), __builtin_bit_cast(unsigned, o[2]),
                             __builtin_bit_cast(unsigned, o[3])};
          __builtin_amdgcn_raw_buffer_store_b128(pv, r_z, (int)vo_z[t], ((rowbase + 8 * m) >> 3) * OHW * 32, 0);
        } else {
          unsigned hi2[2], lo2[2];
#pragma unroll
          for (int k = 0; k < 2; ++k) {
            const float a = o[2 * k] * ASC16, b2 = o[2 * k + 1] * ASC16;
            bad16 |= !(fabsf(a) < 65520.0f) | !(fabsf(b2) < 65520.0f);
            const f32x2_ v2 = {a, b2};
            const f16x2_ hq2 = __builtin_convertvector(v2, f16x2_);
            const f32x2_ back = __builtin_convertvector(hq2, f32x2_);
            const f32x2_ rest = {a - back[0], b2 - back[1]};
            const f16x2_ lq2 = __builtin_convertvector(rest, f16x2_);
            hi2[k] = __builtin_bit_cast(unsigned, hq2);
            lo2[k] = __builtin_bit_cast(unsigned, lq2);
          }
          const u32x2_ hv2 = {hi2[0], hi2[1]}, lv2 = {lo2[0], lo2[1]};
          const int so16 = ((cst + 8 * m) >> 3) * 2 * OHW * 16;
          __builtin_amdgcn_raw_buffer_store_b64(hv2, r_o16, (int)vo_o[t], so16, 0);
          __builtin_amdgcn_raw_buffer_store_b64(lv2, r_o16, (int)vo_o[t], so16 + OHW * 16, 0);
        }
      }
    }
#undef GRU16_FETCH
  }
  if (bad16 && d.guard) atomicOr(d.guard, 1);
}

template <int WC, int WP, int TC, int TP, class PixMap, bool OUT16 = false>
__device__ __forceinline__ void conv_epilogue_px(const accflow_conv_desc& d, f32x16 (&acc)[TC][TP], int cblk0, int wc,
                                                 int wp, int lane, int OHW, PixMap pixmap, int stat_b = 0,
                                                 int stat_slot = 0) {
#define ACCFLOW_EPI_CASE(E, A)                                                                          \
  case (E) * 8 + (A): conv_epilogue_impl<E, A, WC, WP, TC, TP, PixMap, OUT16>(d, acc, cblk0, wc, wp, lane, OHW, pixmap, stat_b, stat_slot); break;
  switch (d.epi * 8 + d.act) {
    ACCFLOW_EPI_CASE(ACCFLOW_EPI_STORE, ACCFLOW_ACT_NONE)
    ACCFLOW_EPI_CASE(ACCFLOW_EPI_STORE, ACCFLOW_ACT_RELU)
    ACCFLOW_EPI_CASE(ACCFLOW_EPI_STORE, ACCFLOW_ACT_SIGMOID)
    ACCFLOW_EPI_CASE(ACCFLOW_EPI_RES_RELU, ACCFLOW_ACT_RELU)
    ACCFLOW_EPI_CASE(ACCFLOW_EPI_RES_RELU, ACCFLOW_ACT_NONE)
    ACCFLOW_EPI_CASE(ACCFLOW_EPI_GRU_ZR, ACCFLOW_ACT_SIGMOID)
    ACCFLOW_EPI_CASE(ACCFLOW_EPI_GRU_Q, ACCFLOW_ACT_TANH)
    ACCFLOW_EPI_CASE(ACCFLOW_EPI_ACCUM, ACCFLOW_ACT_NONE)
    default:
      switch (d.act) {
        case ACCFLOW_ACT_RELU: conv_epilogue_impl<-1, ACCFLOW_ACT_RELU, WC, WP, TC, TP>(d, acc, cblk0, wc, wp, lane, OHW, pixmap); break;
        case ACCFLOW_ACT_SIGMOID: conv_epilogue_impl<-1, ACCFLOW_ACT_SIGMOID, WC, WP, TC, TP>(d, acc, cblk0, wc, wp, lane, OHW, pixmap); break;
        case ACCFLOW_ACT_TANH: conv_epilogue_impl<-1, ACCFLOW_ACT_TANH, WC, WP, TC, TP>(d, acc, cblk0, wc, wp, lane, OHW, pixmap); break;
        default: conv_epilogue_impl<-1, ACCFLOW_ACT_NONE, WC, WP, TC, TP>(d, acc, cblk0, wc, wp, lane, OHW, pixmap);
      }
  }
#undef ACCFLOW_EPI_CASE
}

template <int WC, int WP, int TC, int TP>
__device__ __forceinline__ void conv_epilogue(const accflow_conv_desc& d, f32x16 (&acc)[TC][TP], int cblk0, int wc,
                                              int wp, int lane, int OHW, int Ptot, int ptile) {
  constexpr int BP = WP * TP * 32;
  const int tile0 = ptile * BP;
  const int stat_b = tile0 / OHW, stat_slot = ((tile0 - stat_b * OHW) / BP) * WP + wp;
  accflow_conv_desc e = d;
  if (d.wsplit_bs && d.wscale16) e.wscale16 = d.wscale16 + (long long)stat_b * d.CoutPad;
  conv_epilogue_px<WC, WP, TC, TP>(e, acc, cblk0, wc, wp, lane, OHW, [&](int j, int& b) {
    const int p = tile0 + j;
    if (p >= Ptot) return -1;
    b = p / OHW;
    return p - b * OHW;
  }, stat_b, stat_slot);
}

typedef int i32x4 __attribute__((ext_vector_type(4)));
typedef const __attribute__((address_space(4))) i32x4* ktab_ptr;
__device__ __forceinline__ ktab_ptr as_ktab(const int* p) { return (ktab_ptr)(unsigned long long)p; }

template <int XPT>
__device__ __forceinline__ void gather_x(const XLoaderCtx& c, ktab_ptr ktab, int k0, __amdgpu_buffer_rsrc_t r0,
                                         __amdgpu_buffer_rsrc_t r1, float (&xr)[XPT]) {
  k0 = __builtin_amdgcn_readfirstlane(k0);
  i32x4 e[XPT];
#pragma unroll
  for (int i = 0; i < XPT; ++i) e[i] = ktab[k0 + i];
#pragma unroll
  for (int i = 0; i < XPT; ++i) {
    const int iy = c.iy0 + e[i].y, ix = c.ix0 + e[i].z;
    const bool ok = (unsigned)iy < (unsigned)c.H && (unsigned)ix < (unsigned)c.W;
    const unsigned koff = (unsigned)(e[i].x * c.HW + e[i].y * c.W + e[i].z) * 4u;
    const unsigned off = ok ? (e[i].w ? c.pixbyte1 : c.pixbyte0) + koff : 0xFFFFFFFFu;
    xr[i] = __builtin_bit_cast(float, __builtin_amdgcn_raw_buffer_load_b32(e[i].w ? r1 : r0, (int)off, 0, 0));
  }
}

typedef unsigned u32x4 __attribute__((ext_vector_type(4)));
typedef __bf16 bf16x8 __attribute__((ext_vector_type(8)));
typedef __bf16 bf16x2 __attribute__((ext_vector_type(2)));
typedef float f32x2 __attribute__((ext_vector_type(2)));

typedef _Float16 f16x8 __attribute__((ext_vector_type(8)));
typedef _Float16 f16x2 __attribute__((ext_vector_type(2)));

template <int OFF, int N>
__device__ __forceinline__ void split8_f16(const float (&x)[N], u32x4 (&out)[2], bool& bad, float s) {
  unsigned hi[4], lo[4];
#pragma unroll
  for (int j = 0; j < 4; ++j) {
    const float a = x[OFF + 2 * j] * s, b = x[OFF + 2 * j + 1] * s;
    bad |= !(fabsf(a) < 65520.0f) | !(fabsf(b) < 65520.0f);
    const f32x2 v = {a, b};
// ... 174 lines not shown
```

accflow_amd/networks/raft/update.py:

```python
import torch
import torch.nn as nn

import os

from ... import ops
from .._packs import PackCache, require_cuda

FUSE_LOOKUP = os.environ.get("ACCFLOW_FUSE_LOOKUP", "1") == "1"
USE_H16_STATE = os.environ.get("ACCFLOW_H16_STATE", "1") == "1"


def h16_state_supported():
    return not ops.S16_VIA_MULTI and ops.conv_gru16_supported()


class FlowHead(nn.Module):
    def __init__(self, input_dim=128, hidden_dim=256):
        super().__init__()
        self.conv1 = nn.Conv2d(input_dim, hidden_dim, 3, padding=1)
        self.conv2 = nn.Conv2d(hidden_dim, 2, 3, padding=1)
        self.relu = nn.ReLU(inplace=True)


class SepConvGRU(nn.Module):
    def __init__(self, hidden_dim=128, input_dim=192 + 128):
        super().__init__()
        cin = hidden_dim + input_dim
        for suffix, ks, pad in (("1", (1, 5), (0, 2)), ("2", (5, 1), (2, 0))):
            for gate in "zrq":
                setattr(self, "conv%s%s" % (gate, suffix), nn.Conv2d(cin, hidden_dim, ks, padding=pad))
        self.hidden_dim = hidden_dim
        self.input_dim = input_dim


class BasicMotionEncoder(nn.Module):
    def __init__(self, args):
        super().__init__()
        cor_planes = args.corr_levels * (2 * args.corr_radius + 1) ** 2
        self.convc1 = nn.Conv2d(cor_planes, 256, 1, padding=0)
        self.convc2 = nn.Conv2d(256, 192, 3, padding=1)
        self.convf1 = nn.Conv2d(2, 128, 7, padding=3)
        self.convf2 = nn.Conv2d(128, 64, 3, padding=1)
        self.conv = nn.Conv2d(64 + 192, 128 - 2, 3, padding=1)


class UpdateWorkspace:

    def __init__(self, B, h, w, device, hidden=128, x_dim=256):
        def buf(c):
            return torch.empty((B, c, h, w), dtype=torch.float32, device=device)
        self.B, self.h, self.w, self.hidden, self.x_dim = B, h, w, hidden, x_dim
        self._buf = buf
        self.s16 = bool(ops.s16_active())
        self.net_in_h16 = False
        self.c1_fused = False
        self.descs = {}
        self.hx = buf(hidden + x_dim)
        self.net = self.hx[:, :hidden]
        self.inp = self.hx[:, hidden:hidden + 128]
        self.motion = self.hx[:, hidden + 128:hidden + 256]
        self.motion_conv = self.hx[:, hidden + 128:hidden + 254]
        self.motion_flow = self.hx[:, hidden + 254:hidden + 256]
        self.x = self.hx[:, hidden:]
        self.z = buf(hidden)
        self.flow = buf(2)
        self._corr = None
        if not self.s16:
            self.rh = buf(hidden)
            self.flow16 = buf(16)
            self.c1 = buf(256)
            self.corflo = buf(256)
            self.f1 = buf(128)
            self.head = buf(256)
        self.mask = None
        self.gru_pre = None
        if self.s16:
            def s(c, zero=False):
                return ops.S16.empty(B, c, h, w, device, zero=zero)
            self._corr16 = None
            self.stack16 = s(16)
            self.c1_16, self.corflo16, self.f1_16, self.head16 = s(256), s(256), s(128), s(256)
            self.h16, self.rh16 = s(hidden), s(hidden)
            self.net_in_h16 = USE_H16_STATE and h16_state_supported()
            self.x16 = s(x_dim - 128)
            self.motion16 = self.x16.channels(0, 128)


def _fill_s16_inputs(ws, flow_or_coords, is_flow):
    if not ws.s16:
        return
    B, h, w = ws.B, ws.h, ws.w
    c = ws.corr.view(B, 4, 9, 9, h, w).transpose(2, 3).reshape(B, 4, 81, h, w)
    c88 = torch.zeros((B, 4, 88, h, w), dtype=torch.float32, device=ws.corr.device)
    c88[:, :, :81] = c
    ops.to_s16(c88.view(B, 352, h, w), ws.corr16)
    ops.to_s16(ws.net, ws.h16)
    ops.flow_from_coords_s16(flow_or_coords, ws.flow, ws.motion_flow, ws.stack16, ws.motion16, 126, is_flow=is_flow)


UpdateWorkspace.fill_s16_inputs = _fill_s16_inputs


def _ws_corr(ws):
    if ws._corr is None:
        ws._corr = ws._buf(324)
    return ws._corr


UpdateWorkspace.corr = property(_ws_corr)


def _ws_corr16(ws):
    if ws._corr16 is None:
        ws._corr16 = ops.S16.empty(ws.B, ops.LOOKUP_S16_CHANNELS, ws.h, ws.w, ws.hx.device)
    return ws._corr16


UpdateWorkspace.corr16 = property(_ws_corr16)


def _ws_net32(ws):
    return ws.h16.to_float() if (ws.s16 and ws.net_in_h16) else ws.net.contiguous()


UpdateWorkspace.net32 = _ws_net32


class BasicUpdateBlock(nn.Module):
    def __init__(self, args, hidden_dim=128, input_dim=128):
        super().__init__()
        self.args = args
        self.encoder = BasicMotionEncoder(args)
        self.gru = SepConvGRU(hidden_dim=hidden_dim, input_dim=128 + hidden_dim)
        self.flow_head = FlowHead(hidden_dim, hidden_dim=256)
        self.mask = nn.Sequential(nn.Conv2d(128, 256, 3, padding=1), nn.ReLU(inplace=True),
                                  nn.Conv2d(256, 64 * 9, 1, padding=0))
        self._packs = PackCache()

    def prepack(self):
        pk, e, g, f = self._packs, self.encoder, self.gru, self.flow_head
        pk.conv("c1", e.convc1); pk.conv("c2", e.convc2); pk.conv("f1s", e.convf1, rows_as_channels=True)
        if ops.s16_active():
            pk.conv("c1s", e.convc1, lookup88=True)
            if FUSE_LOOKUP:
                pk.conv("c1f", e.convc1, lookup_fused=True)
        pk.conv("f2", e.convf2)
        pk.conv("cf", e.conv)
        for s in ("1", "2"):
            self._gru_packs(s)
        pk.conv("fh1", f.conv1); pk.conv("fh2", f.conv2)
        pk.conv("m0", self.mask[0]); pk.conv("m2", self.mask[2], const_scale=0.25)

    def motion_encoder(self, ws):
        pk, e = self._packs, self.encoder
        if ws.s16:
            R, D = ops.ACT_RELU, ws.descs
            fused = ws.c1_fused
            if "c2" in D:
                for k in ("c2", "f1", "f2", "cf") if fused else ("c1", "c2", "f1", "f2", "cf"):
                    ops.conv2d(None, None, cache=(D, k))
                return
            if not fused:
                ops.conv2d(pk.conv("c1s", e.convc1, lookup88=True), ws.corr16, out16=ws.c1_16, act=R, fp32_out=False,
                           algo_cin=324, cache=(D, "c1"))
            ops.conv2d(pk.conv("c2", e.convc2), ws.c1_16, out16=ws.corflo16.channels(0, 192), act=R, fp32_out=False,
                       cache=(D, "c2"))
            ops.conv2d(pk.conv("f1s", e.convf1, rows_as_channels=True), ws.stack16, out16=ws.f1_16, act=R, fp32_out=False,
                       algo_cin=2 * 7, cache=(D, "f1"))
            ops.conv2d(pk.conv("f2", e.convf2), ws.f1_16, out16=ws.corflo16.channels(192, 256), act=R, fp32_out=False,
                       cache=(D, "f2"))
            want32 = ws.x_dim > 256
            ops.conv2d(pk.conv("cf", e.conv), ws.corflo16, out16=ws.motion16.channels(0, 126), act=R, fp32_out=want32,
                       out=ws.motion_conv if want32 else None, cache=(D, "cf"))
            return
        ops.conv2d(pk.conv("c1", e.convc1), ws.corr, out=ws.c1, act=ops.ACT_RELU)
        ops.conv2d(pk.conv("c2", e.convc2), ws.c1, out=ws.corflo[:, :192], act=ops.ACT_RELU)
        ops.conv2d(pk.conv("f1s", e.convf1, rows_as_channels=True), ws.flow16, out=ws.f1, act=ops.ACT_RELU, algo_cin=2 * 7)
        ops.conv2d(pk.conv("f2", e.convf2), ws.f1, out=ws.corflo[:, 192:], act=ops.ACT_RELU)
        ops.conv2d(pk.conv("cf", e.conv), ws.corflo, out=ws.motion_conv, act=ops.ACT_RELU)

    def _gru_packs(self, s):
        pk, g, hd = self._packs, self.gru, self.gru.hidden_dim
        cin = hd + g.input_dim
        var, ctx = [(0, hd), (hd + 128, cin)], [(hd, hd + 128)]
        zr = [getattr(g, "convz" + s), getattr(g, "convr" + s)]
        q = [getattr(g, "convq" + s)]
        return (pk.conv_cat("zr%sv" % s, zr, C0=hd, in_slices=var), pk.conv_cat("zr%sc" % s, zr, in_slices=ctx, with_bias=False),
                pk.conv_cat("q%sv" % s, q, C0=hd, in_slices=var), pk.conv_cat("q%sc" % s, q, in_slices=ctx, with_bias=False))

    def gru_context(self, ws):
        B, h, w, hd = ws.B, ws.h, ws.w, ws.hidden
        ws.gru_pre = {}
        inp = ops.to_s16(ws.inp) if ws.s16 else ws.inp
        p32 = ws.s16 and ws.net_in_h16
        for s in ("1", "2"):
            _, zrc, _, qc = self._gru_packs(s)
            ws.gru_pre["zr" + s] = ops.conv2d(zrc, inp, algo_cin=0, p32_out=p32)
            ws.gru_pre["q" + s] = ops.conv2d(qc, inp, algo_cin=0, p32_out=p32)

    def gru_step(self, ws):
        if getattr(ws, "gru_pre", None) is None:
            self.gru_context(ws)
        rest = ws.hx[:, ws.hidden + 128:]
        cin = ws.hidden + ws.x_dim
        if ws.s16:
            D = ws.descs
            if "zr1" in D:
                for k in ("zr1", "q1", "zr2", "q2"):
                    ops.conv2d(None, None, cache=(D, k))
                return
            h16s = ws.net_in_h16
            for s in ("1", "2"):
                zrv, _, qv, _ = self._gru_packs(s)
                ops.conv2d(zrv, ws.h16, in1=ws.x16, out=ws.z, act=ops.ACT_SIGMOID, epi=ops.EPI_GRU_ZR, e0=ws.h16 if h16s else ws.net,
                           out16=ws.rh16, fp32_out=False, pre=ws.gru_pre["zr" + s], algo_cin=cin, cache=(D, "zr" + s))
                ops.conv2d(qv, ws.rh16, in1=ws.x16, out=None if h16s else ws.net, act=ops.ACT_TANH, epi=ops.EPI_GRU_Q,
                           e0=ws.h16 if h16s else ws.net, e1=ws.z, out16=ws.h16, fp32_out=not h16s,
                           pre=ws.gru_pre["q" + s], algo_cin=cin, cache=(D, "q" + s))
            return
        for s in ("1", "2"):
            zrv, _, qv, _ = self._gru_packs(s)
            ops.conv2d(zrv, ws.net, in1=rest, out=ws.z, act=ops.ACT_SIGMOID, epi=ops.EPI_GRU_ZR, e0=ws.net, out2=ws.rh,
                       pre=ws.gru_pre["zr" + s], algo_cin=cin)
            ops.conv2d(qv, ws.rh, in1=rest, out=ws.net, act=ops.ACT_TANH, epi=ops.EPI_GRU_Q, e0=ws.net, e1=ws.z,
                       pre=ws.gru_pre["q" + s], algo_cin=cin)

    def flow_delta(self, ws, coords1=None, out=None):
        pk, f = self._packs, self.flow_head
        if ws.s16:
            D = ws.descs
            if coords1 is not None and ops.profiler.ACTIVE is None and "fh12" in D and D["fh12"][1] is coords1:
                return ops.conv2d_tapgemm(None, None, None, cache=(D, "fh12"))
            p1, p2 = pk.conv("fh1", f.conv1), pk.conv("fh2", f.conv2)
            if ops.tapgemm_eligible(p1, p2, ws.h16):
                if coords1 is not None:
                    return ops.conv2d_tapgemm(p1, p2, ws.h16, out=coords1, epi=ops.EPI_ACCUM, e0=coords1, cache=(D, "fh12"))
                return ops.conv2d_tapgemm(p1, p2, ws.h16, out=out)
            ops.conv2d(p1, ws.h16, out16=ws.head16, act=ops.ACT_RELU, fp32_out=False, cache=(ws.descs, "fh1"))
            if coords1 is not None:
                return ops.conv2d(pk.conv("fh2", f.conv2), ws.head16, out=coords1, epi=ops.EPI_ACCUM, e0=coords1)
            return ops.conv2d(pk.conv("fh2", f.conv2), ws.head16, out=out)
        ops.conv2d(pk.conv("fh1", f.conv1), ws.net, out=ws.head, act=ops.ACT_RELU)
        if coords1 is not None:
            return ops.conv2d(pk.conv("fh2", f.conv2), ws.head, out=coords1, epi=ops.EPI_ACCUM, e0=coords1)
        return ops.conv2d(pk.conv("fh2", f.conv2), ws.head, out=out)

    def up_mask(self, ws):
        pk = self._packs
        if ws.mask is None:
            ws.mask = torch.empty((ws.B, 576, ws.h, ws.w), dtype=torch.float32, device=ws.hx.device)
        if ws.s16:
            ops.conv2d(pk.conv("m0", self.mask[0]), ws.h16, out16=ws.head16, act=ops.ACT_RELU, fp32_out=False)
            return ops.conv2d(pk.conv("m2", self.mask[2], const_scale=0.25), ws.head16, out=ws.mask)
        ops.conv2d(pk.conv("m0", self.mask[0]), ws.net, out=ws.head, act=ops.ACT_RELU)
        return ops.conv2d(pk.conv("m2", self.mask[2], const_scale=0.25), ws.head, out=ws.mask)

    def step(self, ws, coords1, want_mask):
        self.motion_encoder(ws)
        self.gru_step(ws)
        self.flow_delta(ws, coords1=coords1)
        return self.up_mask(ws) if want_mask else None

    @torch.no_grad()
    @ops.range_guarded
    def forward(self, net, inp, corr, flow, upsample=True):
        require_cuda(net, inp, corr, flow)
        B, _, h, w = net.shape
        ws = UpdateWorkspace(B, h, w, net.device)
        ops.copy_into(net.float(), ws.net)
        ops.copy_into(inp.float(), ws.inp)
        ops.copy_into(corr.float(), ws.corr)
        ws.fill_s16_inputs(flow.float().contiguous(), is_flow=True)
        if not ws.s16:
            ops.flow_from_coords(flow.float().contiguous(), dst0=ws.flow, dst1=ws.motion_flow, stack16=ws.flow16, is_flow=True)
        self.motion_encoder(ws)
        self.gru_step(ws)
        delta = self.flow_delta(ws)
        mask = self.up_mask(ws)
        return ws.net32(), mask, delta
```

accflow_amd/ops.py:

```python
import contextlib
import ctypes
import functools
import threading

import torch

from . import _lib, profiler
from ._lib import ConvDesc

import os

ACT_NONE, ACT_RELU, ACT_SIGMOID, ACT_TANH = 0, 1, 2, 3
CONV_F32, CONV_BF16X3, CONV_BF16X6, CONV_F16X3 = 0, 2, 3, 4
_MODES = {"f32": CONV_F32, "bf16x3": CONV_BF16X3, "bf16x6": CONV_BF16X6, "f16x3": CONV_F16X3}
CONV_MODE = _MODES[os.environ.get("ACCFLOW_CONV_MODE", "f16x3").lower()]
_tls = threading.local()


USE_PATCH = os.environ.get("ACCFLOW_CONV_PATCH", "1") == "1"


def set_conv_mode(name):
    global CONV_MODE
    CONV_MODE = _MODES[name.lower()]


def current_mode():
    md = getattr(_tls, "mode", None)
    return CONV_MODE if md is None else md


def conv_mode_name():
    return {v: k for k, v in _MODES.items()}[current_mode()]


class conv_mode:

    def __init__(self, name):
        self.md = _MODES[name.lower()] if isinstance(name, str) else int(name)

    def __enter__(self):
        self.saved = getattr(_tls, "mode", None)
        _tls.mode = self.md

    def __exit__(self, *exc):
        _tls.mode = self.saved

EPI_STORE, EPI_RES_RELU, EPI_GRU_ZR, EPI_GRU_Q, EPI_ACCUM, EPI_TAPGEMM = 0, 1, 2, 3, 4, 5


def _stream():
    return ctypes.c_void_p(torch.cuda.current_stream().cuda_stream)


def _p(t):
    return ctypes.c_void_p(t.data_ptr()) if t is not None else ctypes.c_void_p(0)


def _check(rc, name):
    if rc != 0:
        raise RuntimeError("libaccflow_hip: %s failed with hipError %d" % (name, rc))


def _plane4(t, name):
    if not (isinstance(t, torch.Tensor) and t.is_cuda and t.dtype == torch.float32 and t.dim() == 4):
        raise RuntimeError("%s: expected a 4-D float32 CUDA tensor, got %s" % (
            name, (tuple(t.shape), t.dtype, t.device) if isinstance(t, torch.Tensor) else type(t)))
    B, C, H, W = t.shape
    st = t.stride()
    if not (st[3] == 1 and (H == 1 or st[2] == W) and (C == 1 or st[1] == H * W)):
        raise RuntimeError("%s: channel block must be dense NCHW (strides %s)" % (name, st))
    return st[0] if B > 1 else C * H * W


def _dense(t, name):
    if not (isinstance(t, torch.Tensor) and t.is_cuda and t.dtype == torch.float32 and t.is_contiguous()):
        raise RuntimeError("%s: expected a contiguous float32 CUDA tensor" % name)
    return t


USE_DEFORM_COLUMNS = os.environ.get("ACCFLOW_DEFORM_COLUMNS", "1") == "1"
USE_TAPSUM = os.environ.get("ACCFLOW_CONV_TAPSUM", "1") == "1"
TAPSUM_F16 = os.environ.get("ACCFLOW_TAPSUM_F16", "1") == "1"
PACK_FUSED = os.environ.get("ACCFLOW_PACK_FUSED", "1") == "1"
TAPGEMM_MAXROWS = 18
FUSE_TAPGEMM = os.environ.get("ACCFLOW_FUSE_FLOWHEAD", "1") == "1"
TAPSUM_MIN_PIXELS = 4096
USE_KSPLIT = os.environ.get("ACCFLOW_CONV_KSPLIT", "1") == "1"
KSPLIT_MAX_PIXELS = 4 * 7680


def _ksplit_on():
    return USE_KSPLIT and not getattr(_tls, "no_ksplit", False)


@contextlib.contextmanager
def ksplit_scope(enabled):
    saved = getattr(_tls, "no_ksplit", False)
    _tls.no_ksplit = not enabled
    try:
        yield
    finally:
        _tls.no_ksplit = saved


def _ksplit_ws(n, device):
    store = _tls.__dict__.setdefault("ksplit_ws", {})
    key = (device.index, torch.cuda.current_stream(device).cuda_stream)
    t = store.get(key)
    if t is None or t.numel() < n:
        t = torch.empty(n, dtype=torch.float32, device=device)
        store[key] = t
    return t


def _guard(device):
    scoped = getattr(_tls, "guard_flag", None)
    if scoped is not None:
        return scoped
    store = _tls.__dict__.setdefault("guards", {})
    t = store.get(device.index)
    if t is None:
        t = torch.zeros(1, dtype=torch.int32, device=device)
        store[device.index] = t
    return t


def guard_tripped(device=None, reset=True):
    tripped = False
    for idx, t in getattr(_tls, "guards", {}).items():
        if device is not None and torch.device(device).index not in (None, idx):
# ... 348 lines not shown
    if d.mode == CONV_F16X3 and pk.wscale16 is not None:
        if d.wpatch and pk.wpatch16 is not None:
            d.wpatch16 = pk.wpatch16.data_ptr()
        if pk.wsplit16 is not None:
            d.wsplit16 = pk.wsplit16.data_ptr()
        d.wscale16 = pk.wscale16.data_ptr()
        d.guard = _guard(in0.device).data_ptr()
    if d.wpatch and _ksplit_on() and B * OH * OW <= KSPLIT_MAX_PIXELS and pk.Cout > 4:
        ws = _ksplit_ws(4 * B * pk.Cout * OH * OW, in0.device)
        d.kws, d.kws_elems = ws.data_ptr(), ws.numel()
    if e0 is not None:
        d.e0_bs = _plane4(e0, "e0")
        d.e0 = e0.data_ptr()
    if e1 is not None:
        d.e1_bs = _plane4(e1, "e1")
        d.e1 = e1.data_ptr()
    if out2 is not None:
        d.out2_bs = _plane4(out2, "out2")
        d.out2 = out2.data_ptr()
    if pre is not None:
        if epi not in (EPI_GRU_ZR, EPI_GRU_Q) or tuple(pre.shape) != (B, pk.Cout, OH, OW):
            raise RuntimeError("conv2d: `pre` is a (B, Cout, OH, OW) addend of the GRU epilogues")
        d.pre_bs = _plane4(pre, "pre")
        d.pre = pre.data_ptr()
    if offset is not None:
        d.offset_bs = _plane4(offset, "offset")
        d.offset = offset.data_ptr()
        d.dmask_bs = _plane4(dmask, "dmask")
        d.dmask = dmask.data_ptr()
        if not pk.tap_major:
            raise RuntimeError("deformable conv needs tap-major packed weights")
    if in_norm is not None:
        if in1 is not None or tuple(_dense(in_norm, "in_norm").shape) != (B, C0, 2):
            raise RuntimeError("conv2d: in_norm is (B, C0, 2) for a single-source input")
        if not lib.accflow_conv_in_norm_supported(ctypes.byref(d)):
            return None
        d.in_norm = in_norm.data_ptr()
    if stats_holder is not None and USE_NORM_STATS:
        slots = lib.accflow_conv_stat_slots(ctypes.byref(d))
        if slots > 0:
            st = ConvStats(torch.empty((B, pk.Cout, slots, 3), dtype=torch.float32, device=in0.device), slots)
            d.stats, d.stat_slots = st.partial.data_ptr(), slots
            stats_holder.append(st)
    tm = profiler.ACTIVE
    if tm is not None and tm.wants("conv2d"):
        t0 = tm.begin()
        _check(lib.accflow_conv2d_f32(ctypes.byref(d), _stream()), "accflow_conv2d_f32")
        acin = pk.Cin if algo_cin is None else algo_cin
        tm.end("conv2d", t0, 2.0 * acin * pk.KH * pk.KW * pk.Cout * B * OH * OW,
               "Cin%d Cout%d k%dx%d s%d B%d %dx%d%s%s" % (pk.Cin, pk.Cout, pk.KH, pk.KW, pk.stride, B, OH, OW,
                                                         " deform" if offset is not None else "",
                                                         "" if algo_cin is None else " (stands for Cin%d)" % algo_cin),
               work_exec=2.0 * pk.Cin * pk.KH * pk.KW * pk.Cout * B * OH * OW)
        return out
    _check(lib.accflow_conv2d_f32(ctypes.byref(d), _stream()), "accflow_conv2d_f32")
    return out


def _conv2d_s16(pk, in0, in1, out, act, epi, e0, e1, out2, mode, pre, algo_cin, out16, fp32_out, cache=None, p32_out=False):
    lib = _lib.load()
    md = current_mode() if mode is None else mode
    if md != CONV_F16X3 or (pk.wpatch16 is None and pk.wsplit16 is None):
        raise RuntimeError("conv2d: S16 tensors need the f16x3 mode and a direct-kernel weight pack")
    d = ConvDesc()
    fmt = 0
    srcs = []
    for k, t in enumerate((in0, in1)):
        if t is None:
            srcs.append((None, 0, 0))
        elif isinstance(t, S16):
            fmt |= 1 << k
            srcs.append((t.ptr(), t.bs, t.C))
        else:
            srcs.append((t.data_ptr(), _plane4(t, "in%d" % k), t.shape[1]))
    if fmt and fmt != (3 if in1 is not None else 1):
        raise RuntimeError("conv2d: both sources must have the same format")
    B, _, H, W = in0.shape
    if in1 is not None and (in1.shape[0] != B or tuple(in1.shape[2:]) != (H, W)):
        raise RuntimeError("conv2d: in0/in1 shape mismatch")
    C0, C1 = srcs[0][2], srcs[1][2]
    if C0 != pk.C0 or C0 + C1 != pk.Cin:
        raise RuntimeError("conv2d: channel split (%d,%d) does not match packed weights (C0=%d, Cin=%d)" % (C0, C1, pk.C0, pk.Cin))
    OH, OW = pk.out_size(H, W)
    n_out = pk.Cout // 2 if epi == EPI_GRU_ZR else pk.Cout
    dev = in0.data.device if isinstance(in0, S16) else in0.device
    if out is None and (fp32_out or epi == EPI_GRU_ZR):
        out = torch.empty((B, n_out, OH, OW), dtype=torch.float32, device=dev)
    if out is not None:
        d.out_bs = _plane4(out, "out")
        if tuple(out.shape) != (B, n_out, OH, OW):
            raise RuntimeError("conv2d: out shape %s != %s" % (tuple(out.shape), (B, n_out, OH, OW)))
        d.out = out.data_ptr()
    if out16 is not None:
        if tuple(out16.shape) != (B, n_out, OH, OW):
            raise RuntimeError("conv2d: out16 shape %s != %s" % (out16.shape, (B, n_out, OH, OW)))
        d.out16, d.out16_bs = out16.ptr(), out16.bs
    d.in0, d.in0_bs = srcs[0][0], srcs[0][1]
    d.in1, d.in1_bs = srcs[1][0], srcs[1][1]
    d.in_fmt = fmt
    if S16_VIA_MULTI and fmt:
        d.nsrc = 2 if in1 is not None else 1
        for k in range(d.nsrc):
            S = d.src[k]
            S.ptr, S.bs, S.C, S.Hs, S.Ws = srcs[k][0], srcs[k][1], srcs[k][2], H, W
            S.step, S.oy, S.ox, S.KH, S.KW, S.padH, S.padW = 1, 0, 0, pk.KH, pk.KW, pk.padH, pk.padW
    d.C0, d.C1, d.B, d.H, d.W, d.OH, d.OW = C0, C1, B, H, W, OH, OW
    d.KH, d.KW, d.stride, d.padH, d.padW, d.Cout = pk.KH, pk.KW, pk.stride, pk.padH, pk.padW, pk.Cout
    d.wpack, d.ktab, d.Kpad, d.CoutPad = pk.wpack.data_ptr(), pk.ktab.data_ptr(), pk.Kpad, pk.CoutPad
    d.bias = pk.bias.data_ptr() if pk.bias is not None else None
    d.act, d.epi, d.mode = act, epi, md
    d.wsplit = pk.wsplit.data_ptr() if pk.wsplit is not None else None
    if pk.wpatch16 is not None:
        d.wpatch, d.wpatch16 = pk.wpatch.data_ptr(), pk.wpatch16.data_ptr()
    if pk.wsplit16 is not None:
        d.wsplit16 = pk.wsplit16.data_ptr()
    d.wscale16 = pk.wscale16.data_ptr()
    d.guard = _guard(dev).data_ptr()
    ws_keep = None
    if _ksplit_on() and B * OH * OW <= KSPLIT_MAX_PIXELS and pk.Cout > 4 and not isinstance(e0, S16) and not p32_out:
        ws_keep = _ksplit_ws(4 * B * pk.Cout * OH * OW, dev)
        d.kws, d.kws_elems = ws_keep.data_ptr(), ws_keep.numel()
    if isinstance(e0, S16):
        if epi not in (EPI_GRU_ZR, EPI_GRU_Q) or tuple(e0.shape) != (B, n_out, OH, OW):
            raise RuntimeError("conv2d: an S16 e0 is the GRU epilogues' state operand, shape (B, hidden, OH, OW)")
        d.e0_bs, d.e0, d.e0_fmt = e0.bs, e0.ptr(), 1
        d.p32 = 3 if epi == EPI_GRU_ZR else 6
    elif e0 is not None:
        d.e0_bs, d.e0 = _plane4(e0, "e0"), e0.data_ptr()
    if e1 is not None:
        d.e1_bs, d.e1 = _plane4(e1, "e1"), e1.data_ptr()
    if out2 is not None:
        d.out2_bs, d.out2 = _plane4(out2, "out2"), out2.data_ptr()
    if pre is not None:
        if epi not in (EPI_GRU_ZR, EPI_GRU_Q) or tuple(pre.shape) != (B, pk.Cout, OH, OW):
            raise RuntimeError("conv2d: `pre` is a (B, Cout, OH, OW) addend of the GRU epilogues")
        d.pre_bs, d.pre = _plane4(pre, "pre"), pre.data_ptr()
    if p32_out:
        if epi != EPI_STORE or out is None or pk.Cout % 128 or isinstance(e0, S16):
            raise RuntimeError("conv2d: p32_out is a plain fp32 store onto a multiple of 128 channels")
        d.p32 = 1
    tm = profiler.ACTIVE
    t0 = tm.begin() if tm is not None and tm.wants("conv2d") else None
    _check(lib.accflow_conv2d_f32(ctypes.byref(d), _stream()), "accflow_conv2d_f32 (S16)")
    if t0 is not None:
        acin = pk.Cin if algo_cin is None else algo_cin
        tm.end("conv2d", t0, 2.0 * acin * pk.KH * pk.KW * pk.Cout * B * OH * OW,
               "Cin%d Cout%d k%dx%d s%d B%d %dx%d S16%s%s" % (pk.Cin, pk.Cout, pk.KH, pk.KW, pk.stride, B, OH, OW,
                                                            "in" if fmt else "", "" if algo_cin is None else " (stands for Cin%d)" % algo_cin),
               work_exec=2.0 * pk.Cin * pk.KH * pk.KW * pk.Cout * B * OH * OW)
    ret = out if (out is not None and (fp32_out or out16 is None)) else out16
    if cache is not None and profiler.ACTIVE is None:
        cache[0][cache[1]] = (d, ret, (pk, in0, in1, out, out16, e0, e1, out2, pre, ws_keep))
    return ret



def tapgemm_eligible(pk1, pk2, in0, in1=None):
    if not (FUSE_TAPGEMM and current_mode() == CONV_F16X3 and isinstance(in0, S16) and (in1 is None or isinstance(in1, S16))):
        return False
    B, _, H, W = in0.shape
    nb = B * ((W + 31) // 32) * ((H + 3) // 4) * (pk1.Cout // 128)
    return (pk1.wpatch16 is not None and pk1.Cout % 128 == 0 and pk1.stride == 1 and pk2.ztaps_acc is not None
            and pk2.Cin == pk1.Cout and pk1.out_size(H, W) == (H, W) and not (_ksplit_on() and nb < 320))


def conv2d_tapgemm(pk1, pk2, in0, in1=None, out=None, epi=EPI_STORE, e0=None, cache=None):
    lib = _lib.load()
    if cache is not None and profiler.ACTIVE is None:
        hit = cache[0].get(cache[1])
        if hit is not None:
            _check(lib.accflow_conv2d_f32(ctypes.byref(hit[0]), _stream()), "accflow_conv2d_f32 (tapgemm, cached)")
            _check(lib.accflow_tap_sum_parts_f32(*hit[2], _stream()), "accflow_tap_sum_parts_f32 (cached)")
            return hit[1]
    if pk1 is None:
        raise RuntimeError("conv2d_tapgemm: no packed weights given and no cached descriptor for %r to replay"
                           % (cache[1] if cache is not None else None,))
    if not tapgemm_eligible(pk1, pk2, in0, in1):
        raise RuntimeError("conv2d_tapgemm: shapes / mode outside the fused form (ops.tapgemm_eligible)")
    if epi not in (EPI_STORE, EPI_ACCUM, EPI_RES_RELU) or (epi != EPI_STORE and e0 is None):
        raise RuntimeError("conv2d_tapgemm: epi is STORE, ACCUM (+ e0) or RES_RELU (+ e0)")
    B, _, H, W = in0.shape
    C0, C1 = in0.C, (in1.C if in1 is not None else 0)
    if C0 != pk1.C0 or C0 + C1 != pk1.Cin:
        raise RuntimeError("conv2d_tapgemm: channel split (%d,%d) does not match packed weights" % (C0, C1))
    dev = in0.data.device
    pz = pk2.ztaps_acc
    rows, nparts = pz.Cout, pk1.Cout // 128
    z = torch.empty((nparts, B, rows, H, W), dtype=torch.float32, device=dev)
    if out is None:
        out = torch.empty((B, pk2.Cout, H, W), dtype=torch.float32, device=dev)
    d = ConvDesc()
    d.in0, d.in0_bs = in0.ptr(), in0.bs
    if in1 is not None:
        d.in1, d.in1_bs = in1.ptr(), in1.bs
    d.in_fmt = 3 if in1 is not None else 1
    d.C0, d.C1, d.B, d.H, d.W, d.OH, d.OW = C0, C1, B, H, W, H, W
    d.KH, d.KW, d.stride, d.padH, d.padW, d.Cout = pk1.KH, pk1.KW, 1, pk1.padH, pk1.padW, pk1.Cout
    d.wpack, d.ktab, d.Kpad, d.CoutPad = pk1.wpack.data_ptr(), pk1.ktab.data_ptr(), pk1.Kpad, pk1.CoutPad
    d.bias = pk1.bias.data_ptr() if pk1.bias is not None else None
    d.act, d.epi, d.mode = ACT_RELU, EPI_TAPGEMM, CONV_F16X3
    d.wpatch, d.wpatch16, d.wscale16 = pk1.wpatch.data_ptr(), pk1.wpatch16.data_ptr(), pk1.wscale16.data_ptr()
    d.guard = _guard(dev).data_ptr()
    d.tg_w16, d.tg_scale, d.tg_out = pz.wpatch16.data_ptr(), pz.wscale16.data_ptr(), z.data_ptr()
    d.tg_out_bs, d.tg_out_ps, d.tg_rows, d.tg_coutpad = rows * H * W, B * rows * H * W, rows, pz.CoutPad
    out_bs = _plane4(out, "out")
    e0_bs = _plane4(e0, "e0") if e0 is not None else 0
    targs = (z.data_ptr(), nparts, B * rows * H * W, rows * H * W, _p(pk2.bias) if pk2.bias is not None else None,
             _p(e0) if e0 is not None else None, e0_bs, _p(out), out_bs, B, pk2.Cout, H, W, pk2.KH, pk2.KW, pk2.padH, pk2.padW,
             int(ACT_NONE), int(epi))
    tm = profiler.ACTIVE
    t0 = tm.begin() if tm is not None and tm.wants("conv2d") else None
    _check(lib.accflow_conv2d_f32(ctypes.byref(d), _stream()), "accflow_conv2d_f32 (tapgemm)")
    if t0 is not None:
        px = B * H * W
        tm.end("conv2d", t0, 2.0 * (pk1.Cin * pk1.KH * pk1.KW * pk1.Cout + pk1.Cout * rows) * px,
               "Cin%d Cout%d k%dx%d s1 B%d %dx%d S16in +tapgemm%d" % (pk1.Cin, pk1.Cout, pk1.KH, pk1.KW, B, H, W, rows))
        t0 = tm.begin()
# ... 907 lines not shown
```

include/accflow_hip.h:

```cpp
#ifndef ACCFLOW_HIP_H
#define ACCFLOW_HIP_H

#ifdef __cplusplus
extern "C" {
#endif

#define ACCFLOW_ABI_VERSION 20

enum { ACCFLOW_ACT_NONE = 0, ACCFLOW_ACT_RELU = 1, ACCFLOW_ACT_SIGMOID = 2, ACCFLOW_ACT_TANH = 3 };

enum {
  ACCFLOW_EPI_STORE = 0,
  ACCFLOW_EPI_RES_RELU = 1,
  ACCFLOW_EPI_GRU_ZR = 2,
  ACCFLOW_EPI_GRU_Q = 3,
  ACCFLOW_EPI_ACCUM = 4,
  ACCFLOW_EPI_TAPGEMM = 5
};

enum {
  ACCFLOW_CONV_F32 = 0,
  ACCFLOW_CONV_BF16X3 = 2,
  ACCFLOW_CONV_BF16X6 = 3,
  ACCFLOW_CONV_F16X3 = 4
};
#define ACCFLOW_F16_ASHIFT 4

typedef struct accflow_conv_src {
  const void* ptr;
  long long bs;
  int C, Hs, Ws;
  int step, oy, ox;
  int KH, KW, padH, padW;
  int reserved;
} accflow_conv_src;
#define ACCFLOW_CONV_MAX_SRC 4

typedef struct accflow_conv_desc {
  const float* in0;  const float* in1;
  long long in0_bs, in1_bs;
  int C0, C1;
  int B, H, W;
  int OH, OW;
  int KH, KW, stride, padH, padW;
  int Cout;
  const float* wpack;
  const int*   ktab;
  int Kpad, CoutPad;
  const float* bias;
  float* out;  long long out_bs;
  int act, epi;
  const float* e0; long long e0_bs;
  const float* e1; long long e1_bs;
  float* out2; long long out2_bs;
  const float* offset; long long offset_bs;
  const float* dmask;  long long dmask_bs;
  const void* wsplit;
  int mode;
  const void* wpatch;
  long long wsplit_bs;
  float* kws; long long kws_elems;
  const void* wpatch16; int* guard;
  const float* wscale16;
  const void* wsplit16;
  float* stats; int stat_slots;
  const float* pre; long long pre_bs;
  const float* in_norm;
  float acc_scale;
  int in_fmt;
  void* out16; long long out16_bs;
  int cb;
  long long out_cbs, e0_cbs, out16_cbs;
  int nsrc;
  accflow_conv_src src[ACCFLOW_CONV_MAX_SRC];
  int e0_fmt;
  const void* tg_w16; const float* tg_scale;
  float* tg_out; long long tg_out_bs, tg_out_ps;
  int tg_rows, tg_coutpad;
  int split_c0;
  int p32;
} accflow_conv_desc;

long long accflow_s16_item_words(int C, int H, int W);
int accflow_to_s16_f32(const float* src, long long src_bs, void* dst16, long long dst16_bs, int* guard, int B, int C,
                       int HW, void* stream);

int accflow_conv_kpad(int Cin, int KH, int KW);
int accflow_conv_coutpad(int Cout);

int accflow_conv_pack_f32(const float* w, const float* scale, int Cout, int Cin, int KH, int KW,
                          int C0, int tap_major, float* wpack, int* ktab, void* stream);

int accflow_conv_pack_bf16s(const float* w, const float* scale, int Cout, int Cin, int KH, int KW,
                            void* wsplit, void* stream);

long long accflow_conv_patch_elems(int Cout, int Cin, int KH, int KW);
int accflow_conv_pack_patch(const float* w, const float* scale, int Cout, int Cin, int KH, int KW,
                            void* wpatch, void* stream);
int accflow_conv_pack_patch16(const float* w, const float* scale, int Cout, int Cin, int KH, int KW,
                              void* wpatch16, float* wscale16, void* stream);
// ... 190 lines not shown
```

Measured before the change: 525.6 frame-pairs/s.

## Restructure ConvGRU into r-conv plus fused z,q conv with dual-source gather

Splits each separable ConvGRU half into a conv that computes only r (storing r*h pre-split as fp16) and a fused conv that computes z and q together, gathering both h and r*h patches in one kernel. The z,q conv issues two accumulator tiles per wave over the shared hidden-channel chunks, then finishes z, q and the state blend in a new epilogue that writes the next hidden state directly. This removes the separate fp32 z round-trip and one launch per half, and it ping-pongs between two state buffers. In exchange the kernel uses twice the LDS staging, higher register pressure and an extra z,q weight pack, and it adds alias and size guards.

```diff
diff --git a/accflow_amd/build.py b/accflow_amd/build.py
--- a/accflow_amd/build.py
+++ b/accflow_amd/build.py
@@ -9,7 +9,7 @@
 LIBDIR = os.path.join(HERE, "lib")
 LIB = os.path.join(LIBDIR, "libaccflow_hip.so")
 SOURCES = ["conv2d_f32.hip", "conv2d_f32_v1.hip", "conv2d_f32_v2.hip", "conv2d_f32_v3.hip", "conv2d_bf16s.hip", "conv2d_bf16s_v12.hip", "conv2d_bf16s_v11.hip", "conv2d_bf16s_v21.hip",
-           "conv2d_direct_v_bf16x6.hip", "conv2d_direct_v_bf16n.hip", "conv2d_direct_v_f16.hip", "conv2d_direct_v_s16.hip", "conv2d_direct_v_s16tg.hip", "conv2d_direct_v_s16k.hip", "conv2d_direct_v_s16k9.hip",
+           "conv2d_direct_v_bf16x6.hip", "conv2d_direct_v_bf16n.hip", "conv2d_direct_v_f16.hip", "conv2d_direct_v_s16.hip", "conv2d_direct_v_s16tg.hip", "conv2d_direct_v_s16k.hip", "conv2d_direct_v_s16zq.hip", "conv2d_direct_v_s16k9.hip",
            "conv2d_direct_v_f16n.hip", "conv2d_direct_v_bf16x3.hip", "conv_s16m_v0.hip", "conv_s16m_v1.hip", "conv_s16m_v2.hip",
            "conv_s16m_v3.hip", "conv2d_s16m.hip", "conv_stem.hip", "conv2d_direct.hip", "conv2d.hip", "corr_volume.hip",
            "corr_lookup.hip", "corr_disp.hip", "corr_alt.hip", "corr_lookup_conv.hip", "sampling.hip", "misc.hip", "gma.hip", "backward.hip"]
diff --git a/accflow_amd/csrc/conv2d.hip b/accflow_amd/csrc/conv2d.hip
--- a/accflow_amd/csrc/conv2d.hip
+++ b/accflow_amd/csrc/conv2d.hip
@@ -1,4 +1,6 @@
 #include "conv_common.h"
+#include <initializer_list>
+#include <utility>
 
 namespace {
 
@@ -936,11 +938,28 @@
   dd.acc_scale = 0.0f;
   if (dd.nsrc < 0 || dd.nsrc > ACCFLOW_CONV_MAX_SRC) return 1;
   const bool gru16 = !dd.nsrc && dd.e0_fmt;
+  const bool gru_rzq = dd.epi == ACCFLOW_EPI_GRU_R || dd.epi == ACCFLOW_EPI_GRU_ZQ;
+  if (gru_rzq && !gru16) return 1;
   if (gru16 && !(dd.in_fmt == (dd.in1 ? 3 : 1) && dd.e0 && dd.pre && dd.out16 && dd.mode == ACCFLOW_CONV_F16X3 && !dd.cb && !dd.kws &&
                  dd.KH * dd.KW == 5 && dd.stride == 1 && accflow_conv_gru16_supported() && !dd.stats &&
                  ((dd.epi == ACCFLOW_EPI_GRU_ZR && dd.p32 == 3 && dd.out && dd.Cout == 256) ||
-                  (dd.epi == ACCFLOW_EPI_GRU_Q && dd.p32 == 6 && dd.e1 && dd.Cout == 128))))
+                  (dd.epi == ACCFLOW_EPI_GRU_Q && dd.p32 == 6 && dd.e1 && dd.Cout == 128) ||
+                  (dd.epi == ACCFLOW_EPI_GRU_R && dd.act == ACCFLOW_ACT_SIGMOID && dd.p32 == 2 && !dd.out && !dd.out2 && !dd.e1 &&
+                   dd.Cout == 128) ||
+                  (dd.epi == ACCFLOW_EPI_GRU_ZQ && dd.act == ACCFLOW_ACT_TANH && dd.p32 == 2 && !dd.out && !dd.out2 && dd.e1 &&
+                   dd.Cout == 256 && dd.C0 == 128 && dd.in1 && dd.wpatch16 && dd.wscale16 && dd.B > 0 && dd.H > 0 && dd.W > 0))))
     return 1;
+  if (dd.epi == ACCFLOW_EPI_GRU_ZQ) {
+    const long long item = accflow_s16_item_words(128, dd.H, dd.W) * 4;
+    auto span = [&](const void* p, long long bs) {
+      const char* b = (const char*)p;
+      return std::pair<const char*, const char*>(b, b + ((long long)(dd.B - 1) * bs * 4 + item));
+    };
+    if ((((long long)(dd.B - 1)) * dd.e1_bs) * 4 + item >= (1LL << 32) || dd.e1_bs < 0 || dd.e0_bs < 0 || dd.out16_bs < 0 || dd.in0_bs < 0) return 1;
+    const auto o = span(dd.out16, dd.out16_bs);
+    for (const auto& s : {span(dd.in0, dd.in0_bs), span(dd.e0, dd.e0_bs), span(dd.e1, dd.e1_bs)})
+      if (o.first < s.second && s.first < o.second) return 1;
+  }
   if (!gru16 && dd.p32 && !(dd.p32 == 1 && !dd.nsrc && dd.in_fmt == (dd.in1 ? 3 : 1) && dd.mode == ACCFLOW_CONV_F16X3 && dd.out && !dd.out16 &&
                             dd.epi == ACCFLOW_EPI_STORE && (dd.act == ACCFLOW_ACT_NONE || dd.act == ACCFLOW_ACT_RELU) && !dd.cb &&
                             !dd.kws && !dd.stats && dd.stride == 1 && (dd.Cout % 128) == 0 && accflow_conv_gru16_supported()))
@@ -965,6 +984,8 @@
     return accflow_launch_conv_direct(d, 2, as_stream(stream));
   }
   if (!d.out && (!d.out16 || d.epi == ACCFLOW_EPI_GRU_ZR)) return 1;
+  if (gru_rzq && !(d.Kpad == accflow_conv_kpad(d.C0 + d.C1, d.KH, d.KW) && d.CoutPad == accflow_conv_coutpad(d.Cout) && d.OH == d.H && d.OW == d.W))
+    return 1;
   if (d.epi == ACCFLOW_EPI_GRU_ZR && !d.out2 && !d.out16) return 1;
   if ((d.in_fmt || d.out16) && d.mode != ACCFLOW_CONV_F16X3) return 1;
   if (d.in_fmt & ~3) return 1;
@@ -974,6 +995,7 @@
         ea != ACCFLOW_EPI_STORE * 8 + ACCFLOW_ACT_SIGMOID && ea != ACCFLOW_EPI_RES_RELU * 8 + ACCFLOW_ACT_RELU &&
         ea != ACCFLOW_EPI_RES_RELU * 8 + ACCFLOW_ACT_NONE &&
         ea != ACCFLOW_EPI_GRU_ZR * 8 + ACCFLOW_ACT_SIGMOID && ea != ACCFLOW_EPI_GRU_Q * 8 + ACCFLOW_ACT_TANH &&
+        ea != ACCFLOW_EPI_GRU_R * 8 + ACCFLOW_ACT_SIGMOID && ea != ACCFLOW_EPI_GRU_ZQ * 8 + ACCFLOW_ACT_TANH &&
         ea != ACCFLOW_EPI_ACCUM * 8 + ACCFLOW_ACT_NONE)
       return 1;
   }
@@ -983,7 +1005,7 @@
   if (d.epi == ACCFLOW_EPI_GRU_ZR && (!d.e0 || (d.Cout & 1))) return 1;
   if (d.epi == ACCFLOW_EPI_GRU_ZR && d.out16 && ((d.Cout >> 1) & 7)) return 1;
   if (d.epi == ACCFLOW_EPI_GRU_Q && (!d.e0 || !d.e1)) return 1;
-  if (d.pre && d.epi != ACCFLOW_EPI_GRU_ZR && d.epi != ACCFLOW_EPI_GRU_Q) return 1;
+  if (d.pre && d.epi != ACCFLOW_EPI_GRU_ZR && d.epi != ACCFLOW_EPI_GRU_Q && !gru_rzq) return 1;
   if (d.offset && !d.dmask) return 1;
   if ((long long)d.B * d.OH * d.OW >= (1LL << 31)) return 1;
   if (!multi) {
diff --git a/accflow_amd/csrc/conv2d_direct.hip b/accflow_amd/csrc/conv2d_direct.hip
--- a/accflow_amd/csrc/conv2d_direct.hip
+++ b/accflow_amd/csrc/conv2d_direct.hip
@@ -249,6 +249,10 @@
   if (Z > 1 && (long long)Z * nout > d.kws_elems) Z = (int)(d.kws_elems / nout);
   if (Z < 1) Z = 1;
   if (d.out16 && d.epi == ACCFLOW_EPI_GRU_ZR && ((d.Cout >> 1) & 7)) Z = 1;
+  if (d.epi == ACCFLOW_EPI_GRU_ZQ) {
+    if (TC != 2 || Z != 1 || d.Cout != 256) return 1;
+    return accflow_direct_launch_s16zq(d, dim3((unsigned)((long long)d.B * tiles), 1, 1), st);
+  }
   dim3 grid((unsigned)((long long)d.B * tiles), cdiv(d.Cout, 2 * TC * 32), Z);
   constexpr bool CAN_W4 = TC == 2;
   const bool f16 = d.mode == ACCFLOW_CONV_F16X3 && d.wpatch16;
@@ -697,6 +701,7 @@
 #include "conv2d_direct_v_s16.hip"
 #include "conv2d_direct_v_s16tg.hip"
 #include "conv2d_direct_v_s16k.hip"
+#include "conv2d_direct_v_s16zq.hip"
 #include "conv2d_direct_v_s16k9.hip"
 #include "conv2d_direct_v_f16.hip"
 #include "conv2d_direct_v_f16n.hip"
diff --git a/accflow_amd/csrc/conv2d_direct_kernel.h b/accflow_amd/csrc/conv2d_direct_kernel.h
--- a/accflow_amd/csrc/conv2d_direct_kernel.h
+++ b/accflow_amd/csrc/conv2d_direct_kernel.h
@@ -139,8 +139,9 @@
 
 constexpr int DIR_NORM_MAXC = 256;
 template <int TC, int NT, bool F16 = false, bool W4 = false, bool NORM = false, bool S16 = false, int PM = 7, bool TG = false, int KT = 0,
-          int KWC = 0>
-__global__ __launch_bounds__(256, (KT == 5 ? ACCFLOW_DIRECT_KT_WAVES : 2)) void conv2d_direct_bf16s_kernel(const accflow_conv_desc d) {
+          int KWC = 0, bool ZQ = false>
+__global__ __launch_bounds__(256, (KT == 5 && !ZQ ? ACCFLOW_DIRECT_KT_WAVES : 2)) void conv2d_direct_bf16s_kernel(const accflow_conv_desc d) {
+  static_assert(!ZQ || (W4 && S16 && KT == 5 && !TG), "the z,q form: 4 x 1 wave layout, S16 sources, the 5-tap loop");
   static_assert(!F16 || NT == 2, "the fp16 split has two terms");
   static_assert(KT == 0 || ((S16 || (F16 && NORM)) && (KT & 1)), "the tap-specialised loop: S16 sources or the fp16 normalise-on-load gather, an odd tap count");
   static_assert(!TG || (W4 && S16 && PM == 7), "ACCFLOW_EPI_TAPGEMM: the 4 x 1 wave layout over S16 sources");
@@ -151,12 +152,13 @@
   unsigned long long kp[8] = {0, 0, 0, 0, 0, 0, 0, 0};
 #endif
   constexpr int WC = W4 ? 4 : 2, WP = W4 ? 1 : 2, TP = W4 ? 4 : 2, OCT = 2;
-  constexpr int TCW = W4 ? 1 : TC;
+  constexpr int TCW = ZQ ? 2 : W4 ? 1 : TC;
   constexpr int BC = WC * TCW * 32;
-  static_assert(BC == 2 * TC * 32 && DIR_TH * DIR_TW == WP * TP * 32, "4 x 32 pixel tile = 128 accumulator columns");
+  constexpr int ATILE = ZQ ? 128 : 32;
+  static_assert((ZQ || BC == 2 * TC * 32) && DIR_TH * DIR_TW == WP * TP * 32, "4 x 32 pixel tile = 128 accumulator columns");
   constexpr int PSTAGE = NT * OCT * DIR_NPMAX;
   constexpr int TGWORDS = TG ? 4 * ACCFLOW_TAPGEMM_MAXROWS * DIR_TH * DIR_TW / 4 : 0;
-  __shared__ u32x4 Pst[2 * PSTAGE > TGWORDS ? 2 * PSTAGE : TGWORDS];
+  __shared__ u32x4 Pst[(ZQ ? 4 : 2) * PSTAGE > TGWORDS ? (ZQ ? 4 : 2) * PSTAGE : TGWORDS];
   __shared__ float Nrm[NORM ? 2 * DIR_NORM_MAXC : 2];
 
   const int tid = threadIdx.x, lane = tid & 63;
@@ -231,6 +233,9 @@
   const __amdgpu_buffer_rsrc_t rs16_1 = __builtin_amdgcn_make_buffer_rsrc(
       const_cast<float*>(d.in1 ? d.in1 : d.in0), 0,
       (int)(unsigned)(d.in1 ? (((long long)(d.B - 1)) * d.in1_bs + (long long)O1 * 2 * HW * 4) * 4 : 0), 0x00020000);
+  const __amdgpu_buffer_rsrc_t rs16_2 = __builtin_amdgcn_make_buffer_rsrc(
+      const_cast<float*>(ZQ ? d.e1 : d.in0), 0,
+      (int)(unsigned)(ZQ ? (((long long)(d.B - 1)) * d.e1_bs + (long long)O0 * 2 * HW * 4) * 4 : 0), 0x00020000);
   if constexpr (S16) {
 #pragma unroll
     for (int q = 0; q < 4; ++q) {
@@ -263,6 +268,14 @@
       else
         __builtin_amdgcn_raw_ptr_buffer_load_lds(rs16_0, (__attribute__((address_space(3))) void*)&Pst[slot], 16, (int)voff,
                                                  (int)soff, 0, 0);
+      if constexpr (ZQ) {
+        if (!second) {
+          const unsigned soff2 = (unsigned)__builtin_amdgcn_readfirstlane(
+              (int)((unsigned)((long long)tb * d.e1_bs * 4) + (unsigned)((oct * 2 + t) * HW) * 16u));
+          __builtin_amdgcn_raw_ptr_buffer_load_lds(rs16_2, (__attribute__((address_space(3))) void*)&Pst[slot + 2 * PSTAGE], 16,
+                                                   (int)voff, (int)soff2, 0, 0);
+        }
+      }
     }
   };
   float xa[8], xb[8];
@@ -336,11 +349,11 @@
   const long long step_bytes = 2LL * d.CoutPad * 16, term_bytes = (long long)nstep * step_bytes;
   const __amdgpu_buffer_rsrc_t rsrcw = __builtin_amdgcn_make_buffer_rsrc(const_cast<void*>(F16 ? d.wpatch16 : d.wpatch), 0,
                                                                         (int)(unsigned)(3 * term_bytes), 0x00020000);
-  const unsigned avoff = (unsigned)((kh * d.CoutPad + cblk0 + wc * TCW * 32 + l31) * 16);
+  const unsigned avoff = (unsigned)((kh * d.CoutPad + cblk0 + wc * (ZQ ? 32 : TCW * 32) + l31) * 16);
 #define DIR_LOAD_A(STEP, A)                                                                                      \
   _Pragma("unroll") for (int t = 0; t < NT; ++t) _Pragma("unroll") for (int tc = 0; tc < TCW; ++tc)              \
       A[t][tc] = __builtin_bit_cast(bf16x8, __builtin_amdgcn_raw_buffer_load_b128(                              \
-          rsrcw, (int)(avoff + tc * 512), (int)(unsigned)(t * term_bytes + (STEP) * step_bytes), 0))
+          rsrcw, (int)(avoff + tc * (ATILE * 16)), (int)(unsigned)(t * term_bytes + (STEP) * step_bytes), 0))
 
   int pbase[TP];
 #pragma unroll
@@ -431,16 +444,18 @@
         for (int tc = 0; tc < TCW; ++tc)
         {
           u32x4 frag;
-          s16m_load_a(frag, avoff + tc * 512, wdesc,
+          s16m_load_a(frag, avoff + tc * (ATILE * 16), wdesc,
                       __builtin_amdgcn_readfirstlane((int)(unsigned)(t * term_bytes + (long long)step * step_bytes)));
           A[t][tc] = __builtin_bit_cast(bf16x8, frag);
         }
     };
     constexpr int PWC = DIR_TW + KWC - 1;
     const u32x4* const pb0 = &Pst[kh * DIR_NPMAX + wp * TP * PWC + l31];
-    auto chunk = [&](int cq, bf16x8 (&A0)[NT][TCW], bf16x8 (&A1)[NT][TCW]) __attribute__((always_inline)) {
+    auto chunk = [&](auto dual_, int cq, bf16x8 (&A0)[NT][TCW], bf16x8 (&A1)[NT][TCW]) __attribute__((always_inline)) {
+      constexpr bool DUAL = decltype(dual_)::value;
       const int pstage = cq & 1;
       const bool next_chunk = cq + 1 < c_end;
+      const bool next_dual = ZQ && (cq + 1) * 16 < d.C0;
       const int sbase = cq * KT;
       const u32x4* const pb = pb0 + pstage * PSTAGE;
       dir_static_for<KT>([&](auto tap_) {
@@ -456,34 +471,61 @@
             else gather_patch(cq + 1);
           }
         }
+        constexpr int PA[3] = {1, 0, 0}, PB[3] = {0, 1, 0};
+        if constexpr (DUAL) {
+#pragma unroll
+          for (int tc = 0; tc < TCW; ++tc) {
+            bf16x8 b[NT][TP];
+#pragma unroll
+            for (int tt = 0; tt < NT; ++tt)
+#pragma unroll
+              for (int tp = 0; tp < TP; ++tp)
+                b[tt][tp] = __builtin_bit_cast(bf16x8, pb[tc * 2 * PSTAGE + tt * (OCT * DIR_NPMAX) + tp * PWC + (TAP / KWC) * PWC + TAP % KWC]);
+#pragma unroll
+            for (int pr = 0; pr < 3; ++pr)
+#pragma unroll
+              for (int tp = 0; tp < TP; ++tp) acc[tc][tp] = dir_mfma<F16>(ACUR[PA[pr]][tc], b[PB[pr]][tp], acc[tc][tp]);
+          }
+        } else {
         bf16x8 b[NT][TP];
 #pragma unroll
         for (int tt = 0; tt < NT; ++tt)
 #pragma unroll
           for (int tp = 0; tp < TP; ++tp)
             b[tt][tp] = __builtin_bit_cast(bf16x8, pb[tt * (OCT * DIR_NPMAX) + tp * PWC + (TAP / KWC) * PWC + TAP % KWC]);
-        constexpr int PA[3] = {1, 0, 0}, PB[3] = {0, 1, 0};
 #pragma unroll
         for (int pr = 0; pr < 3; ++pr)
 #pragma unroll
           for (int tc = 0; tc < TCW; ++tc)
 #pragma unroll
             for (int tp = 0; tp < TP; ++tp) acc[tc][tp] = dir_mfma<F16>(ACUR[PA[pr]][tc], b[PB[pr]][tp], acc[tc][tp]);
+        }
 #if ACCFLOW_DIRECT_KT_BUPFRONT
         __builtin_amdgcn_sched_group_barrier(0x100, NT * TP, 0);
         __builtin_amdgcn_sched_group_barrier(0x008, 3 * TCW * TP, 0);
 #endif
         __builtin_amdgcn_sched_barrier(0);
-        if constexpr (TAP == 0 && KT > 1) { if (next_chunk) s16m_wait_vm<NDMA>(); else s16m_wait_vm<0>(); }
+        if constexpr (TAP == 0 && KT > 1) {
+          if (next_dual) s16m_wait_vm<2 * NDMA>(); else if (next_chunk) s16m_wait_vm<NDMA>(); else s16m_wait_vm<0>();
+        }
         else if constexpr (TAP + 1 < KT) { s16m_wait_vm<0>(); }
       });
       s16m_wait_vm<0>();
       if constexpr (!S16) { if (next_chunk) store_patch(pstage ^ 1, cq + 1); }
       __syncthreads();
     };
-    for (int cq = c_begin; cq < c_end; cq += 2) {
-      chunk(cq, aA, aB);
-      if (cq + 1 < c_end) chunk(cq + 1, aB, aA);
+    int cq0 = c_begin;
+    if constexpr (ZQ) {
+      const int nc0 = d.C0 >> 4;
+      for (int cq = 0; cq < nc0; cq += 2) {
+        chunk(std::true_type{}, cq, aA, aB);
+        chunk(std::true_type{}, cq + 1, aB, aA);
+      }
+      cq0 = nc0;
+    }
+    for (int cq = cq0; cq < c_end; cq += 2) {
+      chunk(std::false_type{}, cq, aA, aB);
+      if (cq + 1 < c_end) chunk(std::false_type{}, cq + 1, aB, aA);
     }
   } else {
   for (int step = c_begin * TPC; step < step_end; step += 2) {
@@ -513,6 +555,10 @@
     b = tb;
     return (oy < d.OH && ox < d.OW) ? oy * d.OW + ox : -1;
   };
+  if constexpr (ZQ) {
+    conv_epilogue_gru16zq<TP>(d, acc, wc, lane, OHW, pixmap);
+    return;
+  } else {
   if constexpr (TG) {
     conv_epilogue_tapgemm<F16>(d, acc, cblk0, wave, lane, tid, OHW, pixmap, reinterpret_cast<float*>(Pst));
     return;
@@ -541,12 +587,14 @@
 #endif
   if constexpr (S16 && W4 && KT == 5) {
     if (d.e0_fmt) {
-      if (d.epi == ACCFLOW_EPI_GRU_ZR) conv_epilogue_gru16<true, TP>(d, acc, cblk0, wc, lane, OHW, pixmap);
-      else conv_epilogue_gru16<false, TP>(d, acc, cblk0, wc, lane, OHW, pixmap);
+      if (d.epi == ACCFLOW_EPI_GRU_ZR) conv_epilogue_gru16<1, TP>(d, acc, cblk0, wc, lane, OHW, pixmap);
+      else if (d.epi == ACCFLOW_EPI_GRU_R) conv_epilogue_gru16<2, TP>(d, acc, cblk0, wc, lane, OHW, pixmap);
+      else conv_epilogue_gru16<0, TP>(d, acc, cblk0, wc, lane, OHW, pixmap);
       return;
     }
   }
   conv_epilogue_px<WC, WP, TCW, TP, decltype(pixmap), F16>(d, acc, cblk0, wc, wp, lane, OHW, pixmap, tb, trem * WP + wp);
+  }
 #ifdef ACCFLOW_KPROF
   __builtin_amdgcn_sched_barrier(0);
   const unsigned long long tS = __builtin_amdgcn_s_memrealtime();
@@ -565,6 +613,7 @@
 int accflow_direct_launch_s16tg(const accflow_conv_desc& d, dim3 grid, hipStream_t st);
 int accflow_direct_launch_s16k9(const accflow_conv_desc& d, int tc, bool tapgemm, dim3 grid, hipStream_t st);
 int accflow_direct_launch_s16k(const accflow_conv_desc& d, int kt, dim3 grid, hipStream_t st);
+int accflow_direct_launch_s16zq(const accflow_conv_desc& d, dim3 grid, hipStream_t st);
 int accflow_direct_launch_f16(const accflow_conv_desc& d, int tc, bool w4, dim3 grid, hipStream_t st);
 int accflow_direct_launch_f16_norm(const accflow_conv_desc& d, int tc, dim3 grid, hipStream_t st);
 int accflow_direct_launch_bf16(const accflow_conv_desc& d, int tc, int nt, bool w4, dim3 grid, hipStream_t st);
diff --git a/accflow_amd/csrc/conv2d_direct_v_s16zq.hip b/accflow_amd/csrc/conv2d_direct_v_s16zq.hip
--- /dev/null
+++ b/accflow_amd/csrc/conv2d_direct_v_s16zq.hip
@@ -0,0 +1,12 @@
+#if !defined(ACCFLOW_KPROF) || defined(ACCFLOW_DIRECT_UNITY)
+#include "conv2d_direct_kernel.h"
+int accflow_direct_launch_s16zq(const accflow_conv_desc& d, dim3 grid, hipStream_t st) {
+  if (d.KW == 5 && d.KH == 1)
+    hipLaunchKernelGGL((conv2d_direct_bf16s_kernel<2, 2, true, true, false, true, 7, false, 5, 5, true>), grid, dim3(256), 0, st, d);
+  else if (d.KW == 1 && d.KH == 5)
+    hipLaunchKernelGGL((conv2d_direct_bf16s_kernel<2, 2, true, true, false, true, 7, false, 5, 1, true>), grid, dim3(256), 0, st, d);
+  else
+    return 1;
+  ACCFLOW_RETURN_LAUNCH_STATUS();
+}
+#endif
diff --git a/accflow_amd/csrc/conv_common.h b/accflow_amd/csrc/conv_common.h
--- a/accflow_amd/csrc/conv_common.h
+++ b/accflow_amd/csrc/conv_common.h
@@ -401,10 +401,11 @@
 }
 
 
-template <bool ZR, int TP, class PixMap>
+template <int FORM, int TP, class PixMap>
 __device__ __forceinline__ void conv_epilogue_gru16(const accflow_conv_desc& d, f32x16 (&acc)[1][TP], int cblk0, int wc, int lane,
                                                     int OHW, PixMap pixmap) {
   static_assert(TP == 4, "the 4 x 1 wave layout: 32 channels x 128 pixels per wave");
+  constexpr bool ZR = FORM == 1, SIG = FORM != 0, HAS_Z = FORM == 0;
   constexpr unsigned MASKED = 0xFFFFFFFFu;
   constexpr int TPH = 2;
   typedef float f32x4_ __attribute__((ext_vector_type(4)));
@@ -421,8 +422,9 @@
   const int cst = ZR ? rowbase - half : rowbase;
   auto rng = [&](long long bs, int nch) { return (int)(unsigned)((((long long)(d.B - 1)) * bs + (long long)nch * OHW) * 4); };
   const __amdgpu_buffer_rsrc_t r_pre = __builtin_amdgcn_make_buffer_rsrc(const_cast<float*>(d.pre), 0, rng(d.pre_bs, d.Cout), 0x00020000);
-  const __amdgpu_buffer_rsrc_t r_z = __builtin_amdgcn_make_buffer_rsrc(ZR ? (float*)d.out : const_cast<float*>(d.e1), 0,
-                                                                      ZR ? rng(d.out_bs, half) : rng(d.e1_bs, d.Cout), 0x00020000);
+  const __amdgpu_buffer_rsrc_t r_z = __builtin_amdgcn_make_buffer_rsrc(
+      ZR ? (float*)d.out : HAS_Z ? const_cast<float*>(d.e1) : const_cast<float*>(d.pre), 0,
+      ZR ? rng(d.out_bs, half) : HAS_Z ? rng(d.e1_bs, d.Cout) : 0, 0x00020000);
   const int s16rng = (int)(unsigned)((((long long)(d.B - 1)) * d.e0_bs + (long long)((nst + 7) >> 3) * 2 * OHW * 4) * 4);
   const __amdgpu_buffer_rsrc_t r_h = __builtin_amdgcn_make_buffer_rsrc(const_cast<float*>(d.e0), 0, s16rng, 0x00020000);
   const __amdgpu_buffer_rsrc_t r_o16 = __builtin_amdgcn_make_buffer_rsrc(
@@ -456,7 +458,7 @@
       const int so16_ = ((cst + 8 * (M)) >> 3) * 2 * OHW * 16;                   \
       _Pragma("unroll") for (int t = 0; t < TPH; ++t) {                                                            \
         pre[S][t] = __builtin_bit_cast(f32x4_, __builtin_amdgcn_raw_buffer_load_b128(r_pre, (int)vo_p[t], sop_, 0)); \
-        if (!ZR) zz[S][t] = __builtin_bit_cast(f32x4_, __builtin_amdgcn_raw_buffer_load_b128(r_z, (int)vo_z[t], sop_, 0)); \
+        if (HAS_Z) zz[S][t] = __builtin_bit_cast(f32x4_, __builtin_amdgcn_raw_buffer_load_b128(r_z, (int)vo_z[t], sop_, 0)); \
         if (need_h) {                                                                                              \
           hhi[S][t] = __builtin_bit_cast(u32x2_, __builtin_amdgcn_raw_buffer_load_b64(r_h, (int)vo_h[t], so16_, 0)); \
           hlo[S][t] = __builtin_bit_cast(u32x2_, __builtin_amdgcn_raw_buffer_load_b64(r_h, (int)vo_h[t], so16_ + OHW * 16, 0)); \
@@ -475,12 +477,12 @@
 #pragma unroll
         for (int q = 0; q < 4; ++q) {
           const float v = apply_act(fmaf(acc[0][tp][4 * m + q], sv[S][q], bv[S][q]) + pre[S][t][q],
-                                    ZR ? ACCFLOW_ACT_SIGMOID : ACCFLOW_ACT_TANH);
+                                    SIG ? ACCFLOW_ACT_SIGMOID : ACCFLOW_ACT_TANH);
           if (need_h) {
             const unsigned wh = hhi[S][t][q >> 1], wl = hlo[S][t][q >> 1];
             const unsigned short hq = (unsigned short)((q & 1) ? wh >> 16 : wh & 0xFFFFu), lq = (unsigned short)((q & 1) ? wl >> 16 : wl & 0xFFFFu);
             const float hv = ((float)__builtin_bit_cast(_Float16, hq) + (float)__builtin_bit_cast(_Float16, lq)) * (1.0f / ASC16);
-            o[q] = ZR ? v * hv : gru_blend(zz[S][t][q], hv, v);
+            o[q] = SIG ? v * hv : gru_blend(zz[S][t][q], hv, v);
           } else {
             o[q] = v;
           }
@@ -511,6 +513,101 @@
       }
     }
 #undef GRU16_FETCH
+  }
+  if (bad16 && d.guard) atomicOr(d.guard, 1);
+}
+
+template <int TP, class PixMap>
+__device__ __forceinline__ void conv_epilogue_gru16zq(const accflow_conv_desc& d, f32x16 (&acc)[2][TP], int wc, int lane, int OHW,
+                                                      PixMap pixmap) {
+  static_assert(TP == 4, "the 4 x 1 wave layout: 32 channels x 128 pixels per wave");
+  constexpr unsigned MASKED = 0xFFFFFFFFu;
+  constexpr int TPH = 2;
+  typedef float f32x4_ __attribute__((ext_vector_type(4)));
+  typedef float f32x2_ __attribute__((ext_vector_type(2)));
+  typedef _Float16 f16x2_ __attribute__((ext_vector_type(2)));
+  typedef unsigned u32x2_ __attribute__((ext_vector_type(2)));
+  const int l31 = lane & 31, lh4 = (lane >> 5) * 4;
+  const int half = d.Cout >> 1;
+  const int cst = wc * 32;
+  auto rng = [&](long long bs, int nch) { return (int)(unsigned)((((long long)(d.B - 1)) * bs + (long long)nch * OHW) * 4); };
+  const __amdgpu_buffer_rsrc_t r_pre = __builtin_amdgcn_make_buffer_rsrc(const_cast<float*>(d.pre), 0, rng(d.pre_bs, d.Cout), 0x00020000);
+  const int s16rng_h = (int)(unsigned)((((long long)(d.B - 1)) * d.e0_bs + (long long)((half + 7) >> 3) * 2 * OHW * 4) * 4);
+  const __amdgpu_buffer_rsrc_t r_h = __builtin_amdgcn_make_buffer_rsrc(const_cast<float*>(d.e0), 0, s16rng_h, 0x00020000);
+  const __amdgpu_buffer_rsrc_t r_o16 = __builtin_amdgcn_make_buffer_rsrc(
+      d.out16, 0, (int)(unsigned)((((long long)(d.B - 1)) * d.out16_bs + (long long)((half + 7) >> 3) * 2 * OHW * 4) * 4), 0x00020000);
+  const __amdgpu_buffer_rsrc_t r_b = __builtin_amdgcn_make_buffer_rsrc(const_cast<float*>(d.bias ? d.bias : d.wscale16), 0,
+                                                                      d.bias ? d.Cout * 4 : 0, 0x00020000);
+  const __amdgpu_buffer_rsrc_t r_s = __builtin_amdgcn_make_buffer_rsrc(const_cast<float*>(d.wscale16), 0, d.CoutPad * 4, 0x00020000);
+  constexpr float ASC16 = (float)(1 << ACCFLOW_F16_ASHIFT);
+  bool bad16 = false;
+#pragma unroll
+  for (int hh = 0; hh < TP / TPH; ++hh) {
+    unsigned vo_p[TPH], vo_h[TPH], vo_o[TPH];
+#pragma unroll
+    for (int t = 0; t < TPH; ++t) {
+      int b;
+      const int rem = pixmap((hh * TPH + t) * 32 + l31, b);
+      const bool ok = rem >= 0;
+      vo_p[t] = ok ? (unsigned)((b * d.pre_bs + (long long)rem * 8 + lh4) * 4) : MASKED;
+      vo_h[t] = ok ? (unsigned)((b * d.e0_bs + (long long)rem * 4) * 4 + lh4 * 2) : MASKED;
+      vo_o[t] = ok ? (unsigned)((b * d.out16_bs + (long long)rem * 4) * 4 + lh4 * 2) : MASKED;
+    }
+    f32x4_ prez[2][TPH], preq[2][TPH], bz[2], sz[2], bq[2], sq[2];
+    u32x2_ hhi[2][TPH], hlo[2][TPH];
+#define GRU16ZQ_FETCH(M, S)                                                                                        \
+    do {                                                                                                           \
+      const int cz_ = cst + 8 * (M), cq_ = half + cz_;               \
+      bz[S] = __builtin_bit_cast(f32x4_, __builtin_amdgcn_raw_buffer_load_b128(r_b, (cz_ + lh4) * 4, 0, 0));       \
+      sz[S] = __builtin_bit_cast(f32x4_, __builtin_amdgcn_raw_buffer_load_b128(r_s, (cz_ + lh4) * 4, 0, 0));       \
+      bq[S] = __builtin_bit_cast(f32x4_, __builtin_amdgcn_raw_buffer_load_b128(r_b, (cq_ + lh4) * 4, 0, 0));       \
+      sq[S] = __builtin_bit_cast(f32x4_, __builtin_amdgcn_raw_buffer_load_b128(r_s, (cq_ + lh4) * 4, 0, 0));       \
+      const int so16_ = (cz_ >> 3) * 2 * OHW * 16;                               \
+      _Pragma("unroll") for (int t = 0; t < TPH; ++t) {                                                            \
+        prez[S][t] = __builtin_bit_cast(f32x4_, __builtin_amdgcn_raw_buffer_load_b128(r_pre, (int)vo_p[t], (cz_ >> 3) * OHW * 32, 0)); \
+        preq[S][t] = __builtin_bit_cast(f32x4_, __builtin_amdgcn_raw_buffer_load_b128(r_pre, (int)vo_p[t], (cq_ >> 3) * OHW * 32, 0)); \
+        hhi[S][t] = __builtin_bit_cast(u32x2_, __builtin_amdgcn_raw_buffer_load_b64(r_h, (int)vo_h[t], so16_, 0)); \
+        hlo[S][t] = __builtin_bit_cast(u32x2_, __builtin_amdgcn_raw_buffer_load_b64(r_h, (int)vo_h[t], so16_ + OHW * 16, 0)); \
+      }                                                                                                            \
+    } while (0)
+    GRU16ZQ_FETCH(0, 0);
+#pragma unroll
+    for (int m = 0; m < 4; ++m) {
+      const int S = m & 1;
+      if (m + 1 < 4) GRU16ZQ_FETCH(m + 1, S ^ 1);
+#pragma unroll
+      for (int t = 0; t < TPH; ++t) {
+        const int tp = hh * TPH + t;
+        float o[4];
+#pragma unroll
+        for (int q = 0; q < 4; ++q) {
+          const float zv = apply_act(fmaf(acc[0][tp][4 * m + q], sz[S][q], bz[S][q]) + prez[S][t][q], ACCFLOW_ACT_SIGMOID);
+          const float qv = apply_act(fmaf(acc[1][tp][4 * m + q], sq[S][q], bq[S][q]) + preq[S][t][q], ACCFLOW_ACT_TANH);
+          const unsigned wh = hhi[S][t][q >> 1], wl = hlo[S][t][q >> 1];
+          const unsigned short hq = (unsigned short)((q & 1) ? wh >> 16 : wh & 0xFFFFu), lq = (unsigned short)((q & 1) ? wl >> 16 : wl & 0xFFFFu);
+          const float hv = ((float)__builtin_bit_cast(_Float16, hq) + (float)__builtin_bit_cast(_Float16, lq)) * (1.0f / ASC16);
+          o[q] = gru_blend(zv, hv, qv);
+        }
+        unsigned hi2[2], lo2[2];
+#pragma unroll
+        for (int k = 0; k < 2; ++k) {
+          const float a = o[2 * k] * ASC16, b2 = o[2 * k + 1] * ASC16;
+          bad16 |= !(fabsf(a) < 65520.0f) | !(fabsf(b2) < 65520.0f);
+          const f32x2_ v2 = {a, b2};
+          const f16x2_ hq2 = __builtin_convertvector(v2, f16x2_);
+          const f32x2_ back = __builtin_convertvector(hq2, f32x2_);
+          const f32x2_ rest = {a - back[0], b2 - back[1]};
+          const f16x2_ lq2 = __builtin_convertvector(rest, f16x2_);
+          hi2[k] = __builtin_bit_cast(unsigned, hq2);
+          lo2[k] = __builtin_bit_cast(unsigned, lq2);
+        }
+        const u32x2_ hv2 = {hi2[0], hi2[1]}, lv2 = {lo2[0], lo2[1]};
+        const int so16 = ((cst + 8 * m) >> 3) * 2 * OHW * 16;
+        __builtin_amdgcn_raw_buffer_store_b64(hv2, r_o16, (int)vo_o[t], so16, 0);
+        __builtin_amdgcn_raw_buffer_store_b64(lv2, r_o16, (int)vo_o[t], so16 + OHW * 16, 0);
+      }
+    }
+#undef GRU16ZQ_FETCH
   }
   if (bad16 && d.guard) atomicOr(d.guard, 1);
 }
diff --git a/accflow_amd/networks/raft/update.py b/accflow_amd/networks/raft/update.py
--- a/accflow_amd/networks/raft/update.py
+++ b/accflow_amd/networks/raft/update.py
@@ -53,6 +53,7 @@
         self._buf = buf
         self.s16 = bool(ops.s16_active())
         self.net_in_h16 = False
+        self.gru_rzq = False
         self.c1_fused = False
         self.descs = {}
         self.hx = buf(hidden + x_dim)
@@ -82,6 +83,8 @@
             self.c1_16, self.corflo16, self.f1_16, self.head16 = s(256), s(256), s(128), s(256)
             self.h16, self.rh16 = s(hidden), s(hidden)
             self.net_in_h16 = USE_H16_STATE and h16_state_supported()
+            self.gru_rzq = self.net_in_h16 and hidden == 128
+            self.h16b = s(hidden) if self.gru_rzq else None
             self.x16 = s(x_dim - 128)
             self.motion16 = self.x16.channels(0, 128)
 
@@ -148,6 +151,8 @@
         pk.conv("cf", e.conv)
         for s in ("1", "2"):
             self._gru_packs(s)
+            if ops.s16_active() and USE_H16_STATE and g.hidden_dim == 128 and h16_state_supported():
+                self._gru_packs_rzq(s)
         pk.conv("fh1", f.conv1); pk.conv("fh2", f.conv2)
         pk.conv("m0", self.mask[0]); pk.conv("m2", self.mask[2], const_scale=0.25)
 
@@ -188,9 +193,25 @@
         return (pk.conv_cat("zr%sv" % s, zr, C0=hd, in_slices=var), pk.conv_cat("zr%sc" % s, zr, in_slices=ctx, with_bias=False),
                 pk.conv_cat("q%sv" % s, q, C0=hd, in_slices=var), pk.conv_cat("q%sc" % s, q, in_slices=ctx, with_bias=False))
 
+    def _gru_packs_rzq(self, s):
+        pk, g, hd = self._packs, self.gru, self.gru.hidden_dim
+        cin = hd + g.input_dim
+        var, ctx = [(0, hd), (hd + 128, cin)], [(hd, hd + 128)]
+        r = [getattr(g, "convr" + s)]
+        zq = [getattr(g, "convz" + s), getattr(g, "convq" + s)]
+        return (pk.conv_cat("r%sv" % s, r, C0=hd, in_slices=var), pk.conv_cat("r%sc" % s, r, in_slices=ctx, with_bias=False),
+                pk.conv_cat("zq%sv" % s, zq, C0=hd, in_slices=var), pk.conv_cat("zq%sc" % s, zq, in_slices=ctx, with_bias=False))
+
     def gru_context(self, ws):
         B, h, w, hd = ws.B, ws.h, ws.w, ws.hidden
         ws.gru_pre = {}
+        if ws.s16 and ws.gru_rzq:
+            inp = ops.to_s16(ws.inp)
+            for s in ("1", "2"):
+                _, rc, _, zqc = self._gru_packs_rzq(s)
+                ws.gru_pre["r" + s] = ops.conv2d(rc, inp, algo_cin=0, p32_out=True)
+                ws.gru_pre["zq" + s] = ops.conv2d(zqc, inp, algo_cin=0, p32_out=True)
+            return
         inp = ops.to_s16(ws.inp) if ws.s16 else ws.inp
         p32 = ws.s16 and ws.net_in_h16
         for s in ("1", "2"):
@@ -210,6 +231,14 @@
                     ops.conv2d(None, None, cache=(D, k))
                 return
             h16s = ws.net_in_h16
+            if ws.gru_rzq:
+                for s, src, dst in (("1", ws.h16, ws.h16b), ("2", ws.h16b, ws.h16)):
+                    rv, _, zqv, _ = self._gru_packs_rzq(s)
+                    ops.conv2d(rv, src, in1=ws.x16, act=ops.ACT_SIGMOID, epi=ops.EPI_GRU_R, e0=src, out16=ws.rh16, fp32_out=False,
+                               pre=ws.gru_pre["r" + s], algo_cin=cin, cache=(D, "zr" + s))
+                    ops.conv2d(zqv, src, in1=ws.x16, act=ops.ACT_TANH, epi=ops.EPI_GRU_ZQ, e0=src, e1=ws.rh16, out16=dst,
+                               fp32_out=False, pre=ws.gru_pre["zq" + s], algo_cin=cin, cache=(D, "q" + s))
+                return
             for s in ("1", "2"):
                 zrv, _, qv, _ = self._gru_packs(s)
                 ops.conv2d(zrv, ws.h16, in1=ws.x16, out=ws.z, act=ops.ACT_SIGMOID, epi=ops.EPI_GRU_ZR, e0=ws.h16 if h16s else ws.net,
diff --git a/accflow_amd/ops.py b/accflow_amd/ops.py
--- a/accflow_amd/ops.py
+++ b/accflow_amd/ops.py
@@ -47,6 +47,7 @@
         _tls.mode = self.saved
 
 EPI_STORE, EPI_RES_RELU, EPI_GRU_ZR, EPI_GRU_Q, EPI_ACCUM, EPI_TAPGEMM = 0, 1, 2, 3, 4, 5
+EPI_GRU_R, EPI_GRU_ZQ = 6, 7
 
 
 def _stream():
@@ -561,7 +562,7 @@
     if C0 != pk.C0 or C0 + C1 != pk.Cin:
         raise RuntimeError("conv2d: channel split (%d,%d) does not match packed weights (C0=%d, Cin=%d)" % (C0, C1, pk.C0, pk.Cin))
     OH, OW = pk.out_size(H, W)
-    n_out = pk.Cout // 2 if epi == EPI_GRU_ZR else pk.Cout
+    n_out = pk.Cout // 2 if epi in (EPI_GRU_ZR, EPI_GRU_ZQ) else pk.Cout
     dev = in0.data.device if isinstance(in0, S16) else in0.device
     if out is None and (fp32_out or epi == EPI_GRU_ZR):
         out = torch.empty((B, n_out, OH, OW), dtype=torch.float32, device=dev)
@@ -600,18 +601,24 @@
         ws_keep = _ksplit_ws(4 * B * pk.Cout * OH * OW, dev)
         d.kws, d.kws_elems = ws_keep.data_ptr(), ws_keep.numel()
     if isinstance(e0, S16):
-        if epi not in (EPI_GRU_ZR, EPI_GRU_Q) or tuple(e0.shape) != (B, n_out, OH, OW):
+        if epi not in (EPI_GRU_ZR, EPI_GRU_Q, EPI_GRU_R, EPI_GRU_ZQ) or tuple(e0.shape) != (B, n_out, OH, OW):
             raise RuntimeError("conv2d: an S16 e0 is the GRU epilogues' state operand, shape (B, hidden, OH, OW)")
         d.e0_bs, d.e0, d.e0_fmt = e0.bs, e0.ptr(), 1
-        d.p32 = 3 if epi == EPI_GRU_ZR else 6
+        d.p32 = {EPI_GRU_ZR: 3, EPI_GRU_Q: 6}.get(epi, 2)
     elif e0 is not None:
         d.e0_bs, d.e0 = _plane4(e0, "e0"), e0.data_ptr()
-    if e1 is not None:
+    if epi in (EPI_GRU_R, EPI_GRU_ZQ) and not isinstance(e0, S16):
+        raise RuntimeError("conv2d: EPI_GRU_R / EPI_GRU_ZQ run on the pre-split state only (e0 = an ops.S16)")
+    if epi == EPI_GRU_ZQ:
+        if not isinstance(e1, S16) or tuple(e1.shape) != tuple(in0.shape):
+            raise RuntimeError("conv2d: EPI_GRU_ZQ takes r*h as an ops.S16 `e1` of in0's shape")
+        d.e1_bs, d.e1 = e1.bs, e1.ptr()
+    elif e1 is not None:
         d.e1_bs, d.e1 = _plane4(e1, "e1"), e1.data_ptr()
     if out2 is not None:
         d.out2_bs, d.out2 = _plane4(out2, "out2"), out2.data_ptr()
     if pre is not None:
-        if epi not in (EPI_GRU_ZR, EPI_GRU_Q) or tuple(pre.shape) != (B, pk.Cout, OH, OW):
+        if epi not in (EPI_GRU_ZR, EPI_GRU_Q, EPI_GRU_R, EPI_GRU_ZQ) or tuple(pre.shape) != (B, pk.Cout, OH, OW):
             raise RuntimeError("conv2d: `pre` is a (B, Cout, OH, OW) addend of the GRU epilogues")
         d.pre_bs, d.pre = _plane4(pre, "pre"), pre.data_ptr()
     if p32_out:
diff --git a/include/accflow_hip.h b/include/accflow_hip.h
--- a/include/accflow_hip.h
+++ b/include/accflow_hip.h
@@ -15,7 +15,9 @@
   ACCFLOW_EPI_GRU_ZR = 2,
   ACCFLOW_EPI_GRU_Q = 3,
   ACCFLOW_EPI_ACCUM = 4,
-  ACCFLOW_EPI_TAPGEMM = 5
+  ACCFLOW_EPI_TAPGEMM = 5,
+  ACCFLOW_EPI_GRU_R = 6,
+  ACCFLOW_EPI_GRU_ZQ = 7
 };
 
 enum {
```

After: 529.0 frame-pairs/s, median of 6. Within noise of the previous version (+0.6%).
